# someguynamedjosh/raytrace

Measured on AMD Instinct MI355X. Metric: Mrays/s at 1920x1080 spp=64 (rays actually traced: primary + shadow + diffuse), higher is better.
Workload: dtype f32

## Files before the change

### include/rt_abi.h

```cpp
#ifndef RT_ABI_H
#define RT_ABI_H

#include <stddef.h>
#include <stdint.h>

#ifdef __cplusplus
extern "C" {
#endif

#define RT_CHUNK_SIZE        64
#define RT_MAX_CHUNK_LOD     6
#define RT_ROOT_CHUNK_SIZE   4
#define RT_ROOT_BLOCK_SIZE   256
#define RT_SLICE_SIZE        16
#define RT_SHADER_GROUP_SIZE 8
#define RT_PIXEL_SPREAD      16
#define RT_NOISE_SIZE        512
#define RT_NOISE_BYTES       (512 * 512 * 4)
#define RT_LIGHTING_SCALE    16.0f
#define RT_TRACE_LIMIT       2048
#define RT_NORMAL_AIR        16
#define RT_DEPTH_AIR         0xFFFF
#define RT_MAX_DEPTH         16

// ... 253 lines not shown
typedef struct RtPointLight {
    float    position[3];  float    radius;
    float    color[3];     uint32_t reserved;
} RtPointLight;
int rt_add_lights(RtContext* ctx, const RtUniforms* u, const RtPointLight* lights, uint32_t count);
int rt_add_lights_async(RtContext* ctx, const RtUniforms* u, const RtPointLight* lights_dev, uint32_t count);

int rt_shadow_entities(RtContext* ctx, const RtUniforms* u, const RtDrawBox* boxes, uint32_t nboxes, const RtDrawStamp* models,
                       uint32_t nmodels, float strength);
int rt_shadow_entities_async(RtContext* ctx, const RtUniforms* u, const RtDrawBox* boxes_dev, uint32_t nboxes, const RtDrawStamp* models,
                             uint32_t nmodels, float strength);

int rt_generate_world(RtContext* ctx, uint64_t seed, const int64_t window_lo[3]);
int rt_generate_slice(RtContext* ctx, uint64_t seed, int axis, const int64_t window_lo[3]);

int rt_get_info(RtContext* ctx, RtInfo* out);

uint64_t rt_samples_per_launch(uint64_t lane_bytes, uint64_t npix, uint64_t spp, const char* env_batch);

int rt_upload_noise(RtContext* ctx, const uint8_t* rgba8);

int rt_draw_frame(RtContext* ctx, const RtUniforms* uniforms);

int rt_sync(RtContext* ctx);

int rt_readback(RtContext* ctx, int buffer_id, void* dst, size_t bytes);

size_t rt_buffer_bytes(RtContext* ctx, int buffer_id);

void* rt_device_ptr(RtContext* ctx, int buffer_id);

int rt_set_stream(RtContext* ctx, void* hip_stream);

int rt_tile_count(RtContext* ctx);
int rt_tile_capacity(RtContext* ctx);

int rt_untile(RtContext* ctx, int buffer_id, const void* gathered_dev, int world, void* frame_dev);

void*  rt_gbuffer_ptr(RtContext* ctx);
size_t rt_gbuffer_bytes(RtContext* ctx);
size_t rt_gbuffer_offset(RtContext* ctx, int buffer_id);
int rt_untile_gbuffer(RtContext* ctx, const void* gathered_dev, int world, void* const* frames_dev);

int rt_denoise(RtContext* ctx, int faithful);

int rt_finalize(RtContext* ctx);

int rt_comm_unique_id(void* id_out, size_t bytes);
int rt_comm_init_rank(RtContext* ctx, const void* id, size_t bytes, void** comm_out);
int rt_comm_init_all(int ndev, const int* devices, void** comms_out);
int rt_comm_destroy(void* comm);
int rt_gather_gbuffer(RtContext* ctx, void* comm, int root, void* const* frames_dev, int overlapped);
void* rt_frame_ptr(RtContext* ctx, int buffer_id);
int rt_frame_readback(RtContext* ctx, int buffer_id, void* dst, size_t bytes);

int rt_denoise_planes(RtContext* ctx, void* lighting_rgba16, const void* depth_r16, const void* normal_r8, int faithful);
int rt_finalize_planes(RtContext* ctx, const void* albedo_rgba8, const void* emission_rgba8, const void* fog_rgba8,
                       const void* lighting_rgba16, const void* depth_r16, void* out_bgra8);

typedef struct RtDenoiseParams {
    uint32_t struct_size;
    int32_t  faithful;
    int32_t  weight_by_count;
    uint32_t settle[6];
    uint32_t reserved[3];
} RtDenoiseParams;
int rt_denoise_history(RtContext* ctx, const RtDenoiseParams* params);
int rt_denoise_planes_counted(RtContext* ctx, void* lighting_rgba16, const void* depth_r16, const void* normal_r8,
                              const uint32_t* counts_dev, const RtDenoiseParams* params);

int rt_kernel_in_use(RtContext* ctx);

#define RT_SELFTEST_DENOISE_DIVISION 1
#define RT_SELFTEST_SCENE_MAPS 2
int rt_selftest(RtContext* ctx, int which, uint64_t* result);

int rt_reset_accumulation(RtContext* ctx);
int rt_get_accumulation(RtContext* ctx, uint32_t* frames, uint32_t* samples);
int rt_read_history(RtContext* ctx, uint32_t* counts, size_t bytes);
int rt_edit_boxes_pending(RtContext* ctx, uint32_t* boxes, uint32_t* overflowed);
int rt_slabs_pending(RtContext* ctx, uint32_t* slabs, uint32_t* overflowed);
int rt_read_slab_boxes(RtContext* ctx, float* boxes, uint32_t* count);

int rt_get_counters(RtContext* ctx, RtCounters* out);
int rt_reset_counters(RtContext* ctx);
int rt_get_timing(RtContext* ctx, RtTiming* out);
int rt_get_gather_timing(RtContext* ctx, float* ms_sum, uint32_t* calls);

#define RT_ABI_VERSION_MAJOR 1
#define RT_ABI_VERSION_MINOR 3
uint32_t rt_abi_version(void);

#ifdef __cplusplus
}
#endif
#endif
```

### raytrace_amd/_lib.py

```python
import ctypes as C
import os

from .abi import RtConfig, RtCounters, RtDenoiseParams, RtInfo, RtShapeEdit, RtStampPlace, RtTiming, RtUniforms, RtVoxelEdit

HERE = os.path.dirname(os.path.abspath(__file__))
LIB_AMD_PATH = os.environ.get("RT_AMD_LIB") or os.path.join(HERE, "librt_amd.so")
LIB_HOST_PATH = os.path.join(HERE, "librt_host.so")

ABI_SYMBOLS = (
    "rt_create", "rt_destroy", "rt_last_error", "rt_upload_world", "rt_upload_slice", "rt_slice_staging", "rt_upload_noise",
    "rt_draw_frame", "rt_sync", "rt_readback", "rt_buffer_bytes", "rt_device_ptr", "rt_set_stream",
    "rt_tile_count", "rt_tile_capacity", "rt_untile", "rt_gbuffer_ptr", "rt_gbuffer_bytes", "rt_gbuffer_offset",
    "rt_untile_gbuffer", "rt_denoise", "rt_finalize", "rt_denoise_planes", "rt_finalize_planes", "rt_kernel_in_use", "rt_get_counters", "rt_reset_counters", "rt_get_timing",
    "rt_abi_version",
    "rt_comm_unique_id", "rt_comm_init_rank", "rt_comm_init_all", "rt_comm_destroy", "rt_gather_gbuffer", "rt_frame_ptr",
    "rt_frame_readback", "rt_selftest", "rt_get_info", "rt_samples_per_launch", "rt_get_gather_timing",
    "rt_reset_accumulation", "rt_get_accumulation", "rt_edit_voxels", "rt_read_box",
    "rt_trace_rays", "rt_trace_rays_async", "rt_pick_pixels", "rt_generate_world", "rt_generate_slice", "rt_read_history",
    "rt_edit_boxes_pending", "rt_slabs_pending", "rt_read_slab_boxes", "rt_probe_light", "rt_probe_light_async",
    "rt_denoise_history", "rt_denoise_planes_counted", "rt_sweep_boxes", "rt_sweep_boxes_async",
    "rt_edit_shapes", "rt_draw_boxes", "rt_draw_boxes_async", "rt_add_lights", "rt_add_lights_async",
    "rt_stamp_create", "rt_stamp_capture", "rt_stamp_info", "rt_stamp_read", "rt_stamp_destroy", "rt_edit_stamps",
    "rt_draw_stamps", "rt_draw_stamps_async", "rt_shadow_entities", "rt_shadow_entities_async",
)

_amd = None
_host = None


class NativeLibraryMissing(ImportError):
    pass


def amd():
    global _amd
    if _amd is None:
        if not os.path.exists(LIB_AMD_PATH):
            raise NativeLibraryMissing(
                "%s not found: the HIP extension is required (run `python -m raytrace_amd.build`); "
                "there is no CPU fallback" % LIB_AMD_PATH)
        lib = C.CDLL(LIB_AMD_PATH, mode=C.RTLD_GLOBAL)
        P = C.c_void_p
        lib.rt_create.argtypes = [C.POINTER(RtConfig), C.POINTER(P)]
        lib.rt_create.restype = C.c_int
        lib.rt_destroy.argtypes = [P]
        lib.rt_destroy.restype = None
        lib.rt_last_error.argtypes = [P]
        lib.rt_last_error.restype = C.c_char_p
        lib.rt_upload_world.argtypes = [P, P, P]
        lib.rt_upload_slice.argtypes = [P, C.c_int, C.c_int, P, P]
        lib.rt_slice_staging.argtypes = [P, C.POINTER(P), C.POINTER(P)]
        lib.rt_upload_noise.argtypes = [P, P]
        lib.rt_draw_frame.argtypes = [P, C.POINTER(RtUniforms)]
        lib.rt_sync.argtypes = [P]
        lib.rt_readback.argtypes = [P, C.c_int, P, C.c_size_t]
        lib.rt_buffer_bytes.argtypes = [P, C.c_int]
        lib.rt_buffer_bytes.restype = C.c_size_t
        lib.rt_device_ptr.argtypes = [P, C.c_int]
        lib.rt_device_ptr.restype = P
        lib.rt_set_stream.argtypes = [P, P]
        lib.rt_tile_count.argtypes = [P]
        lib.rt_tile_capacity.argtypes = [P]
        lib.rt_untile.argtypes = [P, C.c_int, P, C.c_int, P]
        lib.rt_gbuffer_ptr.argtypes = [P]
        lib.rt_gbuffer_ptr.restype = P
        lib.rt_gbuffer_bytes.argtypes = [P]
        lib.rt_gbuffer_bytes.restype = C.c_size_t
        lib.rt_gbuffer_offset.argtypes = [P, C.c_int]
        lib.rt_gbuffer_offset.restype = C.c_size_t
        lib.rt_untile_gbuffer.argtypes = [P, P, C.c_int, P]
        lib.rt_untile_gbuffer.restype = C.c_int
        lib.rt_denoise.argtypes = [P, C.c_int]
        lib.rt_finalize.argtypes = [P]
        lib.rt_denoise_planes.argtypes = [P, P, P, P, C.c_int]
        lib.rt_finalize_planes.argtypes = [P, P, P, P, P, P, P]
        lib.rt_denoise_history.argtypes = [P, C.POINTER(RtDenoiseParams)]
        lib.rt_denoise_history.restype = C.c_int
        lib.rt_denoise_planes_counted.argtypes = [P, P, P, P, P, C.POINTER(RtDenoiseParams)]
        lib.rt_denoise_planes_counted.restype = C.c_int
        lib.rt_kernel_in_use.argtypes = [P]
        lib.rt_kernel_in_use.restype = C.c_int
        lib.rt_get_counters.argtypes = [P, C.POINTER(RtCounters)]
        lib.rt_reset_counters.argtypes = [P]
        lib.rt_get_timing.argtypes = [P, C.POINTER(RtTiming)]
        lib.rt_get_info.argtypes = [P, C.POINTER(RtInfo)]
        lib.rt_get_info.restype = C.c_int
        lib.rt_abi_version.restype = C.c_uint32
        lib.rt_samples_per_launch.argtypes = [C.c_uint64, C.c_uint64, C.c_uint64, C.c_char_p]
        lib.rt_samples_per_launch.restype = C.c_uint64
        lib.rt_get_gather_timing.argtypes = [P, C.POINTER(C.c_float), C.POINTER(C.c_uint32)]
        lib.rt_get_gather_timing.restype = C.c_int
        lib.rt_comm_unique_id.argtypes = [P, C.c_size_t]
        lib.rt_comm_init_rank.argtypes = [P, P, C.c_size_t, C.POINTER(P)]
        lib.rt_comm_init_all.argtypes = [C.c_int, C.POINTER(C.c_int), C.POINTER(P)]
        lib.rt_comm_destroy.argtypes = [P]
        lib.rt_gather_gbuffer.argtypes = [P, P, C.c_int, P, C.c_int]
        lib.rt_frame_ptr.argtypes = [P, C.c_int]
        lib.rt_frame_ptr.restype = P
        lib.rt_frame_readback.argtypes = [P, C.c_int, P, C.c_size_t]
        lib.rt_frame_readback.restype = C.c_int
        lib.rt_selftest.argtypes = [P, C.c_int, C.POINTER(C.c_uint64)]
        lib.rt_selftest.restype = C.c_int
        lib.rt_reset_accumulation.argtypes = [P]
        lib.rt_reset_accumulation.restype = C.c_int
        lib.rt_get_accumulation.argtypes = [P, C.POINTER(C.c_uint32), C.POINTER(C.c_uint32)]
        lib.rt_get_accumulation.restype = C.c_int
        lib.rt_read_history.argtypes = [P, P, C.c_size_t]
        lib.rt_read_history.restype = C.c_int
        lib.rt_edit_boxes_pending.argtypes = [P, C.POINTER(C.c_uint32), C.POINTER(C.c_uint32)]
        lib.rt_edit_boxes_pending.restype = C.c_int
        lib.rt_slabs_pending.argtypes = [P, C.POINTER(C.c_uint32), C.POINTER(C.c_uint32)]
        lib.rt_slabs_pending.restype = C.c_int
        lib.rt_read_slab_boxes.argtypes = [P, P, C.POINTER(C.c_uint32)]
        lib.rt_read_slab_boxes.restype = C.c_int
        lib.rt_edit_voxels.argtypes = [P, C.POINTER(RtVoxelEdit), C.c_uint32]
        lib.rt_edit_voxels.restype = C.c_int
        lib.rt_edit_shapes.argtypes = [P, C.POINTER(RtShapeEdit), C.c_uint32]
        lib.rt_edit_shapes.restype = C.c_int
        lib.rt_stamp_create.argtypes = [P, C.POINTER(C.c_int32), P, P, C.POINTER(C.c_uint32)]
        lib.rt_stamp_capture.argtypes = [P, C.POINTER(C.c_int32), C.POINTER(C.c_int32), C.c_uint32, C.POINTER(C.c_uint32)]
        lib.rt_stamp_info.argtypes = [P, C.c_uint32, C.POINTER(C.c_int32)]
        lib.rt_stamp_read.argtypes = [P, C.c_uint32, P, P]
        lib.rt_stamp_destroy.argtypes = [P, C.c_uint32]
        lib.rt_edit_stamps.argtypes = [P, C.POINTER(RtStampPlace), C.c_uint32]
        for name in ("rt_stamp_create", "rt_stamp_capture", "rt_stamp_info", "rt_stamp_read", "rt_stamp_destroy", "rt_edit_stamps"):
            getattr(lib, name).restype = C.c_int
        lib.rt_read_box.argtypes = [P, C.c_int, C.c_int, C.c_int, C.c_int, C.c_int, C.c_int, P, P]
        lib.rt_read_box.restype = C.c_int
        lib.rt_trace_rays.argtypes = [P, P, C.c_uint32, C.POINTER(C.c_int32), P]
        lib.rt_trace_rays.restype = C.c_int
        lib.rt_trace_rays_async.argtypes = [P, P, C.c_uint32, C.POINTER(C.c_int32), P]
        lib.rt_trace_rays_async.restype = C.c_int
        lib.rt_pick_pixels.argtypes = [P, C.POINTER(RtUniforms), P, C.c_uint32, P]
        lib.rt_pick_pixels.restype = C.c_int
        lib.rt_probe_light.argtypes = [P, C.POINTER(RtUniforms), P, C.c_uint32, C.c_uint32, C.c_int32, P]
        lib.rt_probe_light.restype = C.c_int
        lib.rt_probe_light_async.argtypes = [P, C.POINTER(RtUniforms), P, C.c_uint32, C.c_uint32, C.c_int32, P]
        lib.rt_probe_light_async.restype = C.c_int
        lib.rt_sweep_boxes.argtypes = [P, P, C.c_uint32, C.POINTER(C.c_int32), P]
        lib.rt_sweep_boxes.restype = C.c_int
        lib.rt_sweep_boxes_async.argtypes = [P, P, C.c_uint32, C.POINTER(C.c_int32), P]
        lib.rt_sweep_boxes_async.restype = C.c_int
        lib.rt_draw_boxes.argtypes = [P, C.POINTER(RtUniforms), P, P, C.c_uint32]
        lib.rt_draw_boxes.restype = C.c_int
        lib.rt_draw_boxes_async.argtypes = [P, C.POINTER(RtUniforms), P, P, C.c_uint32]
        lib.rt_draw_boxes_async.restype = C.c_int
        lib.rt_draw_stamps.argtypes = [P, C.POINTER(RtUniforms), P, P, C.c_uint32]
        lib.rt_draw_stamps.restype = C.c_int
        lib.rt_draw_stamps_async.argtypes = [P, C.POINTER(RtUniforms), P, P, C.c_uint32]
        lib.rt_draw_stamps_async.restype = C.c_int
        lib.rt_shadow_entities.argtypes = [P, C.POINTER(RtUniforms), P, C.c_uint32, P, C.c_uint32, C.c_float]
        lib.rt_shadow_entities.restype = C.c_int
        lib.rt_shadow_entities_async.argtypes = [P, C.POINTER(RtUniforms), P, C.c_uint32, P, C.c_uint32, C.c_float]
        lib.rt_shadow_entities_async.restype = C.c_int
        lib.rt_add_lights.argtypes = [P, C.POINTER(RtUniforms), P, C.c_uint32]
        lib.rt_add_lights.restype = C.c_int
        lib.rt_add_lights_async.argtypes = [P, C.POINTER(RtUniforms), P, C.c_uint32]
        lib.rt_add_lights_async.restype = C.c_int
        lib.rt_generate_world.argtypes = [P, C.c_uint64, C.POINTER(C.c_int64)]
        lib.rt_generate_world.restype = C.c_int
        lib.rt_generate_slice.argtypes = [P, C.c_uint64, C.c_int, C.POINTER(C.c_int64)]
        lib.rt_generate_slice.restype = C.c_int
        for name in ("rt_comm_unique_id", "rt_comm_init_rank", "rt_comm_init_all", "rt_comm_destroy", "rt_gather_gbuffer"):
            getattr(lib, name).restype = C.c_int
        for name in ("rt_upload_world", "rt_upload_slice", "rt_slice_staging", "rt_upload_noise", "rt_draw_frame", "rt_sync", "rt_readback",
                     "rt_set_stream", "rt_tile_count", "rt_tile_capacity", "rt_untile", "rt_untile_gbuffer", "rt_denoise", "rt_finalize",
                     "rt_denoise_planes", "rt_finalize_planes", "rt_get_counters",
                     "rt_reset_counters", "rt_get_timing"):
            getattr(lib, name).restype = C.c_int
        _amd = lib
    return _amd


def host():
    global _host
    if _host is None:
        amd()
        if not os.path.exists(LIB_HOST_PATH):
            raise NativeLibraryMissing("%s not found (run `python -m raytrace_amd.build`)" % LIB_HOST_PATH)
        lib = C.CDLL(os.environ.get("RT_HOST_LIB") or LIB_HOST_PATH)
        P = C.c_void_p
        lib.rth_material_pack.argtypes = [C.c_int]
        lib.rth_material_pack.restype = C.c_uint32
        lib.rth_material_unpack.argtypes = [C.c_uint32, P, P]
        lib.rth_material_get.argtypes = [C.c_int, P, P, P]
        lib.rth_pack_chunk.argtypes = [P, P, P]
        lib.rth_generate_region.argtypes = [C.c_uint64, P, P]
        lib.rth_generate_region_r.argtypes = [C.c_uint64, C.c_int, P, P]
        lib.rth_region_from_ids.argtypes = [P, P, P]
        lib.rth_heightmap.argtypes = [C.c_long, C.c_long, C.c_uint64, P]
        lib.rth_copy_3d_u32.argtypes = [P] * 7
        lib.rth_copy_3d_auto_clip_u32.argtypes = [P, C.c_int, P, P, C.c_int]
        lib.rth_copy_3d_bounded_auto_clip_u32.argtypes = [P] * 7
        lib.rth_fill_slice_3d_auto_clip_u8.argtypes = [C.c_uint8, P, C.c_int, P, P]
        lib.rth_chunk_codec_available.restype = C.c_int
        lib.rth_chunk_file_name.argtypes = [C.c_long, C.c_long, C.c_long, P]
        lib.rth_chunk_write.argtypes = [C.c_char_p, P, P]
        lib.rth_chunk_read.argtypes = [C.c_char_p, P, P]
        lib.rth_chunk_storage_new.argtypes = [C.c_char_p, C.c_uint64]
        lib.rth_chunk_storage_new.restype = P
        lib.rth_chunk_storage_free.argtypes = [P]
        lib.rth_chunk_storage_free.restype = None
        lib.rth_chunk_storage_borrow.argtypes = [P, C.c_long, C.c_long, C.c_long, P, P]
        lib.rth_chunk_storage_stats.argtypes = [P, P, P]
        lib.rth_tum_new.argtypes = [C.c_uint64]
        lib.rth_tum_new.restype = P
        lib.rth_tum_new_r.argtypes = [C.c_uint64, C.c_int]
        lib.rth_tum_new_r.restype = P
        lib.rth_tum_free.argtypes = [P]
        lib.rth_tum_free.restype = None
        lib.rth_tum_request.argtypes = [P, C.c_int, C.c_int]
# ... 55 lines not shown
```

### raytrace_amd/csrc/api/api_context.hip

```cpp
#include <new>

#include "rt_context.hpp"

using namespace rta;

namespace rta __attribute__((visibility("hidden"))) {

thread_local std::string g_create_error = "";

rtd::Scene scene_of(const RtContext* c) {
    rtd::Scene s;
    s.mine = c->d_mine_sw; s.mat = c->d_mat_sw; s.coarse = c->d_coarse; s.noise = c->d_noise;
    s.brick = c->d_brick ? reinterpret_cast<const uint8_t*>(c->d_brick) : reinterpret_cast<const uint8_t*>(c->d_coarse);
    return s;
}

rtd::Planes planes_of(void* const* planes) {
    rtd::Planes p;
    p.lighting_rgba16 = (uint16_t*)planes[RT_BUF_LIGHTING_RGBA16];
    p.depth_r16 = (uint16_t*)planes[RT_BUF_DEPTH_R16UI];
    p.normal_r8 = (uint8_t*)planes[RT_BUF_NORMAL_R8UI];
    p.albedo_rgba8 = (uint32_t*)planes[RT_BUF_ALBEDO_RGBA8];
    p.emission_rgba8 = (uint32_t*)planes[RT_BUF_EMISSION_RGBA8];
    p.fog_rgba8 = (uint32_t*)planes[RT_BUF_FOG_RGBA8];
    p.lighting_f32 = (float*)planes[RT_BUF_LIGHTING_F32];
    p.fog_f32 = (float*)planes[RT_BUF_FOG_F32];
    p.depth_f32 = (float*)planes[RT_BUF_DEPTH_F32];
    return p;
}

hipError_t join_lanes_into(RtContext* c, hipStream_t st) {
    for (int l = 0; l < c->nlanes; l++) {
        Lane& ln = c->lanes[l];
        if (ln.stream == st || !ln.stream) continue;
        hipError_t e = hipEventRecord(ln.ev_join, ln.stream);
        if (e == hipSuccess) e = hipStreamWaitEvent(st, ln.ev_join, 0);
        if (e != hipSuccess) return e;
    }
    return hipSuccess;
}
hipError_t fence_lanes_after(RtContext* c, hipStream_t st) {
    if (c->nlanes < 2) return hipSuccess;
    hipError_t e = hipEventRecord(c->ev_fence, st);
    for (int l = 0; l < c->nlanes && e == hipSuccess; l++)
        if (c->lanes[l].stream != st) e = hipStreamWaitEvent(c->lanes[l].stream, c->ev_fence, 0);
    return e;
}
hipError_t sync_lanes(RtContext* c) {
    hipError_t e = hipStreamSynchronize(c->stream);
    if (e == hipSuccess && c->query_stream) e = hipStreamSynchronize(c->query_stream);
    for (int l = 0; l < c->nlanes && e == hipSuccess; l++)
        if (c->lanes[l].stream && c->lanes[l].stream != c->stream) e = hipStreamSynchronize(c->lanes[l].stream);
    return e;
}

void invalidate_prepass(RtContext* c) {
    for (FrameSlot& fs : c->slots) fs.prepass_valid = false;
}

void plane_written(RtContext* c, const void* ptr) {
    const uint8_t* q = static_cast<const uint8_t*>(ptr);
    for (int sl = 0; sl < c->nslots; sl++)
        for (int b = 0; b < RT_BUF_COUNT; b++) {
            if (b == RT_BUF_FINAL_BGRA8) continue;
            const uint8_t* base = static_cast<const uint8_t*>(c->slots[sl].planes[b]);
            if (base && q >= base && q < base + c->plane_pixels * kBytesPerPixel[b]) c->slots[sl].prepass_valid = false;
        }
}

}

constexpr uint64_t kDefaultLightBytes = 16ull << 30;
uint64_t rt_light_budget_bytes(const char* env_gib) {
    uint64_t light_bytes = kDefaultLightBytes;
    size_t free_b = 0, total_b = 0;
    if (hipMemGetInfo(&free_b, &total_b) == hipSuccess) { if ((uint64_t)free_b / 10u < light_bytes) light_bytes = (uint64_t)free_b / 10u; }
    else (void)hipGetLastError();
    uint64_t gib = 0;
    if (parse_knob(env_gib, 1, 128, &gib)) light_bytes = gib << 30;
    return light_bytes;
}
extern "C" uint64_t rt_samples_per_launch(uint64_t lane_bytes, uint64_t npix, uint64_t spp, const char* env_batch) {
    if (npix == 0) npix = 1;
    uint64_t B = lane_bytes / (sizeof(rtd::PathLight) * npix);
    if (B > (1ull << 31) / npix) B = (1ull << 31) / npix;
    parse_knob(env_batch, 1, (long long)B - 1, &B);
    if (B < 1) B = 1;
    if (B > spp) B = spp;
    return B;
}

namespace {

int create_device(RtContext* c) {
    RT_HIP(c, hipSetDevice(c->device));
    hipDeviceProp_t prop;
    RT_HIP(c, hipGetDeviceProperties(&prop, c->device));
    c->num_cus = prop.multiProcessorCount > 0 ? prop.multiProcessorCount : 256;
    int reserve = 0;
    if (env_int("RT_RESERVE_CUS", 1, c->num_cus - 1, &reserve)) c->num_cus -= reserve;
    RT_HIP(c, new_stream(c, &c->own_stream));
    c->stream = c->own_stream;
    c->lanes[0].stream = c->own_stream;
    for (hipEvent_t* ev : {&c->ev_frame0, &c->ev_frame1}) RT_HIP(c, new_event(c, ev, hipEventDefault));
    RT_HIP(c, dev_alloc(c, &c->d_mine_sw, c->vox)); RT_HIP(c, dev_alloc(c, &c->d_mat_sw, c->vox));
    RT_HIP(c, dev_alloc(c, &c->d_coarse, (size_t)rtd::kCoarseWords));
    if (c->logr > 8 && getenv("RT_BRICK_MAP")) RT_HIP(c, dev_alloc(c, &c->d_brick, c->vox / 128u / 4u));
    RT_HIP(c, dev_alloc(c, &c->d_noise, (size_t)RT_NOISE_SIZE * RT_NOISE_SIZE));
    RT_HIP(c, dev_alloc(c, &c->d_flag, 4));
    RT_HIP(c, dev_alloc(c, &c->d_counters, 1));
    RT_HIP(c, hipMemset(c->d_counters, 0, sizeof(rtd::DevCounters)));
    return RT_OK;
}

int create_slots(RtContext* c) {
    if (c->nlanes == 2) RT_HIP(c, new_stream(c, &c->lanes[1].stream));
    for (int l = 0; l < c->nlanes; l++) RT_HIP(c, new_event(c, &c->lanes[l].ev_join));
    for (hipEvent_t* ev : {&c->ev_fence, &c->ev_world.ev, &c->ev_query.ev, &c->ev_gather.ev}) RT_HIP(c, new_event(c, ev));
    size_t off = 0;
    for (int b = 0; b <= RT_BUF_FOG_RGBA8; b++) {
        c->gbuffer_offset[b] = off;
        off += (c->plane_pixels * kBytesPerPixel[b] + 255) / 256 * 256;
    }
    c->gbuffer_bytes = off;
    for (int sl = 0; sl < c->nslots; sl++) {
        FrameSlot& fs = c->slots[sl];
        uint8_t* block = nullptr;
        RT_HIP(c, dev_alloc(c, &block, off));
        RT_HIP(c, hipMemset(block, 0, off));
        fs.gbuffer = block;
        for (int b = 0; b <= RT_BUF_FOG_RGBA8; b++) fs.planes[b] = block + c->gbuffer_offset[b];
        for (int b = RT_BUF_FOG_RGBA8 + 1; b < RT_BUF_COUNT; b++) {
            uint8_t* p = nullptr;
            RT_HIP(c, dev_alloc(c, &p, c->plane_pixels * kBytesPerPixel[b]));
            RT_HIP(c, hipMemset(p, 0, c->plane_pixels * kBytesPerPixel[b]));
            fs.planes[b] = p;
        }
        for (hipEvent_t* ev : {&fs.ev_prepass, &fs.ev_acc, &fs.ev_tail.ev}) RT_HIP(c, new_event(c, ev));
    }
    c->cur_slot = 0;
    c->gbuffer = c->slots[0].gbuffer;
    for (int b = 0; b < RT_BUF_COUNT; b++) c->planes[b] = c->slots[0].planes[b];
    return RT_OK;
}

int create_persistent(RtContext* c) {
    const RtConfig& cfg = c->cfg;
    const size_t stack_words = (size_t)4 * c->num_cus * 1024 * (size_t)(cfg.depth > 1 ? cfg.depth - 1 : 1);
    for (int l = 0; l < c->nlanes; l++) {
        Lane& ln = c->lanes[l];
        RT_HIP(c, dev_alloc(c, &ln.cursor, kCursorWords));
        RT_HIP(c, hipMemset(ln.cursor, 0, kCursorWords * sizeof(uint32_t)));
        ln.cursor_clean = true;
        RT_HIP(c, dev_alloc(c, &ln.pstack, stack_words));
    }
    for (int sl = 0; sl < c->nslots; sl++) {
        FrameSlot& fs = c->slots[sl];
        RT_HIP(c, dev_alloc(c, &fs.wl_count, 2 * kWlSetWords));
        RT_HIP(c, hipMemset(fs.wl_count, 0, 2 * kWlSetWords * sizeof(uint32_t)));
        fs.wl_clean[0] = fs.wl_clean[1] = true;
        RT_HIP(c, dev_alloc(c, &fs.worklist, (size_t)c->npix_pad));
        RT_HIP(c, dev_alloc(c, &fs.phit, (size_t)c->npix_pad));
        RT_HIP(c, dev_alloc(c, &fs.pacc, (size_t)c->npix_pad));
    }
    RT_HIP(c, dev_alloc(c, &c->sphere_lut, (size_t)65536));
    RT_HIP(c, dev_alloc(c, &c->sun_lut, (size_t)2 * 65536));
    RT_HIP(c, dev_alloc(c, &c->dif_lut, (size_t)4 * 6 * 65536));
    const uint64_t np = c->npix_pad ? c->npix_pad : 1;
    c->light_budget_bytes = rt_light_budget_bytes(getenv("RT_PERSIST_LIGHT_GIB"));
    uint64_t B = rt_samples_per_launch(c->light_budget_bytes / (uint64_t)c->nlanes, np, (uint64_t)cfg.spp, getenv("RT_PERSIST_BATCH"));
    for (int l = 0; l < c->nlanes; l++) {
        for (;;) {
            const hipError_t e = dev_alloc(c, &c->lanes[l].ppl, (size_t)np * B);
            if (e == hipSuccess) break;
            if (e != hipErrorOutOfMemory || B == 1 || l > 0) RT_HIP(c, e);
            (void)hipGetLastError();
            B = (B + 1) / 2;
        }
    }
    c->persist_batch = (uint32_t)B;
    if (cfg.flags & RT_FLAG_ACCUMULATE) {
        RT_HIP(c, dev_alloc(c, &c->d_accum, (size_t)c->npix_pad));
        RT_HIP(c, new_event(c, &c->ev_accum.ev));
    }
    if (c->reproject) {
        c->d_hist_sum[0] = c->d_accum;
        RT_HIP(c, dev_alloc(c, &c->d_hist_sum[1], (size_t)c->npix_pad));
        for (int h = 0; h < 2; h++) {
            RT_HIP(c, dev_alloc(c, &c->d_hist_rec[h], (size_t)c->npix_pad));
            RT_HIP(c, hipMemset(c->d_hist_rec[h], 0, (size_t)c->npix_pad * sizeof(uint2)));
        }
    }
    if (c->stream_history) {
        RT_HIP(c, dev_alloc(c, &c->d_slab_masks, (size_t)rtd::kSlabSlots * rtd::kSlabSlotWords));
        RT_HIP(c, dev_alloc(c, &c->d_slab_boxes, 1));
        RT_HIP(c, hipMemset(c->d_slab_boxes, 0, sizeof(rtd::SlabBoxes)));
    }
    RT_HIP(c, rtd::launch_sphere_lut(c->sphere_lut, c->own_stream));
    RT_HIP(c, rtd::launch_dif_lut(c->sphere_lut, c->dif_lut, c->own_stream));
    RT_HIP(c, hipStreamSynchronize(c->own_stream));
    return RT_OK;
}

int create_wavefront(RtContext* c) {
    WavefrontState& w = c->wave;
    uint64_t target = 4u << 20;
    env_int("RT_BATCH_PATHS", 1, LLONG_MAX, &target);
    uint64_t B = c->npix_pad ? target / c->npix_pad : 1;
    if (B < 1) B = 1;
    if (B > (uint64_t)c->cfg.spp) B = (uint64_t)c->cfg.spp;
    w.batch_samples = (uint32_t)B;
    uint64_t cap64 = (uint64_t)c->npix_pad * B;
    if (cap64 >= (1ull << 31)) return fail(c, RT_ERR_INVALID_ARG, "rt_create: batch too large");
    w.cap = (uint32_t)cap64;
    const size_t cap = w.cap;
    rtd::ShadeArgs& sa = w.shade;
    RT_HIP(c, dev_alloc(c, &sa.qox, cap)); RT_HIP(c, dev_alloc(c, &sa.qoy, cap)); RT_HIP(c, dev_alloc(c, &sa.qoz, cap));
    RT_HIP(c, dev_alloc(c, &sa.qdx, 2 * cap)); RT_HIP(c, dev_alloc(c, &sa.qdy, 2 * cap)); RT_HIP(c, dev_alloc(c, &sa.qdz, 2 * cap));
    RT_HIP(c, dev_alloc(c, &sa.qid, cap));
    rtd::TraceArgs& ta = w.trace;
    RT_HIP(c, dev_alloc(c, &ta.hx, cap)); RT_HIP(c, dev_alloc(c, &ta.hy, cap)); RT_HIP(c, dev_alloc(c, &ta.hz, cap));
    RT_HIP(c, dev_alloc(c, &ta.hinfo, cap));
    RT_HIP(c, dev_alloc(c, &ta.sunres, cap)); RT_HIP(c, dev_alloc(c, &sa.pnormal, cap)); RT_HIP(c, dev_alloc(c, &sa.pstate, cap));
    RT_HIP(c, dev_alloc(c, &sa.pdx, cap)); RT_HIP(c, dev_alloc(c, &sa.pdy, cap)); RT_HIP(c, dev_alloc(c, &sa.pdz, cap));
    RT_HIP(c, dev_alloc(c, &sa.plx, cap)); RT_HIP(c, dev_alloc(c, &sa.ply, cap)); RT_HIP(c, dev_alloc(c, &sa.plz, cap));
    RT_HIP(c, dev_alloc(c, &sa.sunbits, cap));
    RT_HIP(c, dev_alloc(c, &sa.stack, cap * (size_t)(c->cfg.depth > 1 ? c->cfg.depth - 1 : 1)));
    RT_HIP(c, dev_alloc(c, &w.acc, (size_t)c->npix_pad));
    RT_HIP(c, dev_alloc(c, &w.ctrl, (size_t)2 * (RT_MAX_DEPTH + 2)));
    ta.qox = sa.qox; ta.qoy = sa.qoy; ta.qoz = sa.qoz; ta.qdx = sa.qdx; ta.qdy = sa.qdy; ta.qdz = sa.qdz; ta.qid = sa.qid;
    sa.hx = ta.hx; sa.hy = ta.hy; sa.hz = ta.hz; sa.hinfo = ta.hinfo; sa.sunres = ta.sunres;
    ta.qcap = sa.qcap = sa.npaths_cap = w.cap;
    ta.npix_pad = sa.npix_pad = c->npix_pad;
    ta.refill_threshold = w.refill_threshold;
    ta.counters = sa.counters = c->d_counters;
    return RT_OK;
}
}

extern "C" {

uint32_t rt_abi_version(void) { return ((uint32_t)RT_ABI_VERSION_MAJOR << 16) | (uint32_t)RT_ABI_VERSION_MINOR; }

const char* rt_last_error(RtContext* ctx) { return ctx ? ctx->err.c_str() : g_create_error.c_str(); }

int rt_create(const RtConfig* cfg, RtContext** out) {
    if (out) *out = nullptr;
    if (!cfg || !out) return fail(nullptr, RT_ERR_INVALID_ARG, "rt_create: null argument");
    if (cfg->struct_size != sizeof(RtConfig)) return fail(nullptr, RT_ERR_INVALID_ARG, "rt_create: RtConfig.struct_size mismatch");
    if (cfg->width <= 0 || cfg->height <= 0 || cfg->width > 16384 || cfg->height > 16384)
        return fail(nullptr, RT_ERR_INVALID_ARG, "rt_create: width/height out of range");
    if (cfg->region != 256 && cfg->region != 512 && cfg->region != 1024)
        return fail(nullptr, RT_ERR_INVALID_ARG, "rt_create: region must be 256 (the reference), 512 or 1024");
    if (cfg->region != 256 && cfg->kernel == RT_KERNEL_WAVEFRONT)
        return fail(nullptr, RT_ERR_INVALID_ARG, "rt_create: the split wavefront baseline supports region 256 only");
    if (cfg->spp < 1 || cfg->spp > RT_NOISE_BYTES) return fail(nullptr, RT_ERR_INVALID_ARG, "rt_create: spp out of range");
    if (cfg->depth < 0 || cfg->depth > RT_MAX_DEPTH) return fail(nullptr, RT_ERR_INVALID_ARG, "rt_create: depth out of range");
    if (cfg->tile_world < 1 || cfg->tile_rank < 0 || cfg->tile_rank >= cfg->tile_world)
        return fail(nullptr, RT_ERR_INVALID_ARG, "rt_create: bad tile_rank/tile_world");
    if (cfg->kernel < RT_KERNEL_DEFAULT || cfg->kernel > RT_KERNEL_FRAME || cfg->kernel == 4  ||
        cfg->kernel == 6 )
        return fail(nullptr, RT_ERR_INVALID_ARG, "rt_create: unknown kernel");
    if ((cfg->flags & RT_FLAG_ACCUMULATE) && (cfg->kernel == RT_KERNEL_MEGA || cfg->kernel == RT_KERNEL_WAVEFRONT))
        return fail(nullptr, RT_ERR_UNIMPLEMENTED, "rt_create: RT_FLAG_ACCUMULATE needs RT_KERNEL_DEFAULT, FRAME, PATHS or PERSISTENT (not the baselines)");
    if (cfg->flags & RT_FLAG_REPROJECT) {
        if (!(cfg->flags & RT_FLAG_ACCUMULATE))
            return fail(nullptr, RT_ERR_INVALID_ARG, "rt_create: RT_FLAG_REPROJECT needs RT_FLAG_ACCUMULATE");
        if (cfg->history_cap < 0 || cfg->history_cap > 65535)
            return fail(nullptr, RT_ERR_INVALID_ARG, "rt_create: history_cap must be 0 (the default, 32) or 1..65535");
        if (cfg->edit_radius < 0 || cfg->edit_radius > 64)
            return fail(nullptr, RT_ERR_INVALID_ARG, "rt_create: edit_radius must be 0 (an edit restarts the history) or 1..64");
        if (cfg->stream_history != 0 && cfg->stream_history != 1)
            return fail(nullptr, RT_ERR_INVALID_ARG, "rt_create: stream_history must be 0 (a slab restarts the history) or 1");
        if (cfg->stream_history == 1 && cfg->edit_radius < 1)
            return fail(nullptr, RT_ERR_INVALID_ARG, "rt_create: stream_history = 1 needs edit_radius in 1..64 (its near test uses it)");
        if (cfg->spp != 1 || cfg->tile_world != 1)
            return fail(nullptr, RT_ERR_UNIMPLEMENTED, "rt_create: RT_FLAG_REPROJECT needs one-sample whole frames (spp == 1, tile_world == 1)");
    }

// ... 232 lines not shown
```

### raytrace_amd/csrc/api/api_frame.hip

```cpp
#include "rt_context.hpp"

using namespace rta;

namespace rta __attribute__((visibility("hidden"))) {

void resolve_route(RtContext* c) {
    Route& r = c->route;
    if (r.family != RT_KERNEL_PERSISTENT) { r.in_use = r.family; return; }
    const RtConfig& cfg = c->cfg;
    const int kernel = cfg.kernel;
    const bool cache = (cfg.flags & RT_FLAG_CACHE_PRIMARY) != 0;
    const uint32_t spp = (uint32_t)cfg.spp, B = c->persist_batch;
    const uint64_t npix = c->npix_pad;
    rtd::Frame f{};
    f.depth = cfg.depth; f.logr = c->logr;
    const bool small = spp == 1u ? npix < c->frame_crossover
                                 : npix * spp * (uint64_t)(cfg.depth > 1 ? cfg.depth : 1) < c->frame_crossover_multi;
    r.frame = (cache || spp == 1u) && rtd::launch_frame_ok(f) && spp <= B && !((cfg.flags & RT_FLAG_ACCUMULATE) && spp > 1u) &&
              (kernel == RT_KERNEL_FRAME || (kernel == RT_KERNEL_DEFAULT && small));
    if (cache && kernel != RT_KERNEL_PERSISTENT)
        r.paths_from = kernel != RT_KERNEL_DEFAULT ? 0u : npix == 0 ? UINT32_MAX : (uint32_t)((kPathsCrossover + npix - 1) / npix);
    r.direct = spp == 1u && (!r.on_paths(1) || rtd::launch_paths_direct_ok(f));
    r.threshold_persist = c->persist_threshold ? c->persist_threshold : 32u;
    r.threshold_paths = c->persist_threshold ? c->persist_threshold : (cfg.depth > 4 && c->region == 256) ? 40u : 36u;
// ... 91 lines not shown
    FrameSlot* fs = nullptr;
    rtd::Planes pl{};
    bool one_lane = false;
    Lane* L0 = nullptr;
    hipStream_t st0 = nullptr;
    hipStream_t tail = nullptr;
    uint32_t* wlc = nullptr;
    bool reuse = false;
    bool accum = false, accum_cont = false;
    uint32_t key[16] = {};
    uint64_t accum_n = 0;
    float4* accum_multi = nullptr;
    int temporal_mode = rtd::TEMPORAL_RESTART;
    uint32_t nbox = 0;
    rtd::TemporalBox boxes[rtd::kTemporalMaxBoxes];
    uint32_t nslab = 0;
    int32_t lr_prev[3] = {}, lr[3] = {};
};

rtd::TemporalBox world_box(const EditBox& b, const int32_t lr[3], int region) {
    rtd::TemporalBox w;
    const int64_t R = region;
    for (int k = 0; k < 3; k++) {
        const int64_t base = (int64_t)lr[k] - R / 2;
        const int64_t lo = base + ((((int64_t)b.lo[k] - lr[k]) % R) + R) % R, hi = base + ((((int64_t)b.hi[k] - lr[k]) % R) + R) % R;
        w.lo[k] = (float)(lo <= hi ? lo : base);
        w.hi[k] = (float)(lo <= hi ? hi + 1 : base + R);
    }
    return w;
}

hipError_t frame_begin(RtContext* c, PersistFrame& p, const RtUniforms* u, bool frame_events) {
    p.count = (c->cfg.flags & RT_FLAG_COUNTERS) != 0;
    p.cache = (c->cfg.flags & RT_FLAG_CACHE_PRIMARY) != 0;
    p.nl = c->user_stream ? 1 : c->nlanes;
    p.nsl = c->user_stream ? 1 : c->nslots;
    hipError_t e = hipSuccess;
    if (c->frame_recorded) e = c->slots[c->cur_slot].ev_tail.record(c->stream);
    p.si = p.nsl == 2 ? (int)(c->frames_drawn & 1u) : 0;
    p.fs = &c->slots[p.si];
    p.pl = planes_of(p.fs->planes);
    p.one_lane = p.nsl == 1 && (uint32_t)c->cfg.spp <= c->persist_batch;
    p.L0 = &c->lanes[p.one_lane ? 0u : c->path_launches % (uint64_t)p.nl];
    p.st0 = p.tail = p.L0->stream;
    accum_key_of(u, p.key);
    p.reuse = c->prepass_reuse && p.cache && !c->route.frame && !p.count && c->d_accum == nullptr && !c->reproject &&
              (c->cfg.flags & (RT_FLAG_ACCUMULATE | RT_FLAG_REPROJECT)) == 0 && p.fs->prepass_valid &&
              memcmp(p.key, p.fs->prepass_key, sizeof(p.key)) == 0;
    p.wlc = p.fs->wl_count + kWlSetWords * (size_t)(p.fs->wl_parity ^ (p.reuse ? 1 : 0));
    const uint32_t spp = (uint32_t)c->cfg.spp;
    p.accum = c->d_accum != nullptr;
    if (c->edit_overflow) c->accum_valid = false;
    p.nbox = c->edit_nbox;
    for (uint32_t b = 0; b < p.nbox; b++) p.boxes[b] = world_box(c->edit_boxes[b], u->lr, c->region);
    c->edit_nbox = 0;
    c->edit_overflow = false;
    if (c->slab_overflow) c->accum_valid = false;
    p.nslab = c->slab_pending;
    memcpy(p.lr_prev, &c->accum_key[13], 12); memcpy(p.lr, u->lr, 12);
    c->slab_pending = 0;
    c->slab_overflow = false;
    c->slab_boxes_drawn = false;
    p.accum_cont = p.accum && c->accum_valid && memcmp(p.key, c->accum_key, sizeof(p.key)) == 0 && c->accum_samples + spp <= (1ull << 24);
    p.accum_n = p.accum_cont ? c->accum_samples + spp : spp;
    p.accum_multi = p.accum && spp > 1u ? c->d_accum : nullptr;
    if (c->reproject) {
        const bool still = p.accum_cont;
        const bool same_camera = memcmp(p.key, c->accum_key, sizeof(p.key)) == 0;
        if (still) p.temporal_mode = rtd::TEMPORAL_STILL;
        else if (c->accum_valid && !same_camera && p.key[0] == c->accum_key[0]) p.temporal_mode = rtd::TEMPORAL_MOVED;
        else p.temporal_mode = rtd::TEMPORAL_RESTART;
        if (p.temporal_mode != rtd::TEMPORAL_RESTART && p.nbox > 0u) p.temporal_mode = rtd::TEMPORAL_MOVED_BOXES;
        if (p.temporal_mode != rtd::TEMPORAL_RESTART && p.nslab > 0u) p.temporal_mode = rtd::TEMPORAL_MOVED_SLABS;
        if (p.temporal_mode != rtd::TEMPORAL_RESTART && p.temporal_mode != rtd::TEMPORAL_STILL) {
            p.accum_cont = true;
            p.accum_n = (c->accum_samples < c->history_cap ? c->accum_samples : (uint64_t)c->history_cap) + 1u;
        }
    }
    if (e == hipSuccess) e = p.fs->ev_tail.wait(p.st0);
    if (e == hipSuccess && frame_events) e = hipEventRecord(c->ev_frame0, p.st0);
    return e;
}

hipError_t frame_prepass(RtContext* c, PersistFrame& p) {
    FrameSlot& fs = *p.fs;
    const bool prepass_clears = c->primary_version == 2 && c->npix_pad != 0;
    hipError_t e = hipSuccess;
    fs.prepass_valid = false;
    if (!fs.wl_clean[fs.wl_parity]) e = hipMemsetAsync(p.wlc, 0, kWlClearWords * sizeof(uint32_t), p.st0);
    fs.wl_clean[fs.wl_parity] = false;
    LaunchTimer t(c, 1, p.st0);
    rtd::PrimaryArgs pr{};
    pr.phit = fs.phit;
    pr.worklist = fs.worklist; pr.wl_count = p.wlc; pr.tile_cursor = p.wlc + 32; pr.acc = fs.pacc; pr.counters = c->d_counters;
    const bool clear_cursors = prepass_clears && !p.L0->cursor_clean;
    pr.zero_words = prepass_clears ? fs.wl_count + kWlSetWords * (size_t)(fs.wl_parity ^ 1) : nullptr; pr.zero_count = (uint32_t)kWlClearWords;
    pr.zero_words2 = clear_cursors ? p.L0->cursor : nullptr; pr.zero_count2 = (uint32_t)kCursorWords;
    rtd::Frame fpre = p.f;
    if (p.accum_multi) fpre.spp = 1;
    if (e == hipSuccess) e = rtd::launch_primary(scene_of(c), fpre, p.pl, pr, p.count, c->primary_version, c->num_cus, p.st0);
    if (e == hipSuccess && p.accum_multi) e = c->ev_accum.wait_elsewhere(p.st0);
    if (e == hipSuccess && p.accum_multi)
        e = rtd::launch_accumulate_frame(p.f, p.pl, c->d_accum, c->npix_pad, p.accum_cont, (int)p.accum_n, c->cfg.spp, true, p.st0);
    if (prepass_clears && e == hipSuccess) { fs.wl_clean[fs.wl_parity ^ 1] = true; p.L0->cursor_clean = true; }
    fs.wl_parity ^= 1;
    if (e == hipSuccess) { fs.prepass_valid = true; memcpy(fs.prepass_key, p.key, sizeof(p.key)); }
    return e;
}

hipError_t frame_tables(RtContext* c, PersistFrame& p) {
    const float lut_key[6] = {p.f.sunangle[0], p.f.sunangle[1], p.f.sunangle[2], p.f.sunlight[0], p.f.sunlight[1], p.f.sunlight[2]};
    if (c->cfg.depth < 1 || (c->lut_valid && memcmp(lut_key, c->lut_key, sizeof(lut_key)) == 0)) return hipSuccess;
    hipError_t e = p.nl == 2 ? join_lanes_into(c, p.st0) : hipSuccess;
    {
        LaunchTimer t(c, 1, p.st0);
        if (e == hipSuccess) e = rtd::launch_sun_lut(p.f, c->sun_lut, p.st0);
        if (e == hipSuccess) e = rtd::launch_sky_lut(p.f, c->dif_lut, p.st0);
    }
    if (e == hipSuccess && p.nl == 2) e = fence_lanes_after(c, p.st0);
    c->lut_valid = e == hipSuccess;
    memcpy(c->lut_key, lut_key, sizeof(lut_key));
    return e;
}

hipError_t frame_one_launch(RtContext* c, PersistFrame& p) {
    if (p.nsl == 2) c->path_launches++;
    rtd::FrameArgs fa{};
    fa.threshold = c->frame_threshold; fa.tiles_per_group = c->frame_tiles; fa.sun_lut = c->sun_lut; fa.dif_lut = c->dif_lut; fa.pl = p.L0->ppl; fa.counters = c->d_counters;
    if (getenv("RT_DEBUG_WAVE_DUMP") && (size_t)c->ntiles_local * 32u <= (size_t)4 * c->num_cus * 1024 * sizeof(uint32_t))
        fa.dbg_waves = reinterpret_cast<unsigned long long*>(c->lanes[0].pstack);
    LaunchTimer t(c, 0, p.st0);
    return rtd::launch_frame(scene_of(c), p.f, p.pl, fa, p.count, c->num_cus, p.st0);
}

hipError_t frame_path_batches(RtContext* c, PersistFrame& p) {
    const Route& r = c->route;
    FrameSlot& fs = *p.fs;
    const uint32_t spp = (uint32_t)c->cfg.spp, B = c->persist_batch;
    hipError_t e = hipSuccess;
    if (p.nl == 2 && spp > B) e = hipEventRecord(fs.ev_prepass, p.st0);
    for (uint32_t s0 = 0; s0 < spp && e == hipSuccess; s0 += B) {
        const uint32_t ns = spp - s0 < B ? spp - s0 : B;
        Lane* L = &c->lanes[p.one_lane ? 0u : c->path_launches % (uint64_t)p.nl];
        const hipStream_t st = L->stream;
        if (!p.one_lane) c->path_launches++;
        if (st != p.st0 && s0 == B) e = hipStreamWaitEvent(st, fs.ev_prepass, 0);
        if (e == hipSuccess && !L->cursor_clean) e = hipMemsetAsync(L->cursor, 0, kCursorWords * sizeof(uint32_t), st);
        L->cursor_clean = false;
        const bool to_paths = r.on_paths(ns);
        rtd::PersistArgs pa{};
        pa.cursor = L->cursor; pa.worklist = fs.worklist; pa.wl_count = p.wlc; pa.direct = r.direct ? 1u : 0u;
        pa.npix_pad = c->npix_pad; pa.sample0 = s0; pa.nsamples = ns; pa.chunk = c->persist_chunk;
        pa.threshold = to_paths ? r.threshold_paths : r.threshold_persist;
        pa.nthreads = (uint32_t)c->num_cus * 1024u; pa.stack = L->pstack;
        pa.phit = fs.phit;
        pa.sun_lut = c->sun_lut; pa.dif_lut = c->dif_lut;
        pa.pl = L->ppl; pa.counters = c->d_counters;
        const uint64_t record_bytes = (uint64_t)c->npix_pad * ns * sizeof(rtd::PathLight);
        const bool big_records = record_bytes > kStreamRecordBytes;
        const bool stream_st = c->pl_stream_mode < 0 ? big_records : (c->pl_stream_mode & 1) != 0;
        const bool stream_ld = c->pl_stream_mode < 0 ? big_records : (c->pl_stream_mode & 2) != 0;
        pa.pl_stream = stream_st ? 1u : 0u;
        if (e == hipSuccess) {
            LaunchTimer t(c, 0, st);
            e = to_paths ? rtd::launch_paths(scene_of(c), p.f, p.pl, pa, p.count, c->num_cus, st)
                         : rtd::launch_persist(scene_of(c), p.f, p.pl, pa, p.count, p.cache, 1, c->num_cus, st);
        }
        if (e == hipSuccess && !r.direct) {
            if (p.nl == 2 && s0 != 0) e = hipStreamWaitEvent(st, fs.ev_acc, 0);
            if (e == hipSuccess && p.accum_multi && !p.cache && s0 == 0) e = c->ev_accum.wait_elsewhere(st);
            {
                LaunchTimer t(c, 1, st);
                if (e == hipSuccess)
                    e = rtd::launch_accumulate_paths(p.f, p.pl, L->ppl, fs.worklist, p.wlc, c->npix_pad, ns, s0 == 0, s0 + B >= spp, p.cache,
                                                     stream_ld, fs.pacc, p.accum_multi, p.accum_cont, (int)p.accum_n, L->cursor,
                                                     (uint32_t)kCursorWords, st);
                if (e == hipSuccess && c->npix_pad != 0) L->cursor_clean = true;
            }
            if (e == hipSuccess && p.nl == 2 && s0 + B < spp) e = hipEventRecord(fs.ev_acc, st);
        }
        p.tail = st;
    }
    return e;
}

hipError_t frame_accumulate_tail(RtContext* c, PersistFrame& p) {
    hipError_t e = hipSuccess;
    if (c->cfg.spp == 1) {
        e = c->ev_accum.wait_elsewhere(p.tail);
        LaunchTimer t(c, 1, p.tail);
        if (e == hipSuccess && !c->reproject)
            e = rtd::launch_accumulate_frame(p.f, p.pl, c->d_accum, c->npix_pad, p.accum_cont, (int)p.accum_n, 1, false, p.tail);
        if (e == hipSuccess && c->reproject) {
            rtd::TemporalArgs ta{};
            const int prev = c->hist_cur, next = prev ^ 1;
            ta.prev_sum = c->d_hist_sum[prev]; ta.prev_rec = c->d_hist_rec[prev];
            ta.next_sum = c->d_hist_sum[next]; ta.next_rec = c->d_hist_rec[next];
            memcpy(ta.origin, &c->accum_key[1], 12); memcpy(ta.forward, &c->accum_key[4], 12);
            memcpy(ta.up, &c->accum_key[7], 12); memcpy(ta.right, &c->accum_key[10], 12);
            ta.cap = c->history_cap;
            if (p.temporal_mode == rtd::TEMPORAL_MOVED_SLABS) {
                e = rtd::launch_place_slab_boxes(c->d_slab_masks, p.nslab, p.lr_prev, p.lr, c->logr, c->d_slab_boxes, p.tail);
                ta.slab = c->d_slab_boxes;
                c->slab_boxes_drawn = e == hipSuccess;
            }
            if (p.temporal_mode == rtd::TEMPORAL_MOVED_BOXES || p.temporal_mode == rtd::TEMPORAL_MOVED_SLABS) {
                ta.nbox = p.nbox;
                memcpy(ta.box, p.boxes, sizeof(ta.box));
                ta.r2 = (float)(c->edit_radius * c->edit_radius);
                for (int k = 0; k < 3; k++) { ta.sun[k] = p.f.sunangle[k]; ta.inv_sun[k] = 1.0f / p.f.sunangle[k]; }
            }
            if (e == hipSuccess) e = rtd::launch_temporal_frame(p.f, p.pl, ta, p.temporal_mode, p.tail);
            c->hist_cur = next;
        }
    }
    if (e == hipSuccess && p.nl == 2) e = c->ev_accum.record(p.tail);
    return e;
}

void frame_publish(RtContext* c, const PersistFrame& p, hipError_t e) {
    if (e != hipSuccess) invalidate_prepass(c);
    if (p.accum) {
        c->accum_valid = e == hipSuccess;
        c->accum_frames = p.accum_cont ? c->accum_frames + 1u : 1u;
        c->accum_samples = p.accum_n;
        memcpy(c->accum_key, p.key, sizeof(p.key));
    }
    c->stream = p.tail;
    c->cur_slot = p.si;
    c->gbuffer = p.fs->gbuffer;
    for (int b = 0; b < RT_BUF_COUNT; b++) c->planes[b] = p.fs->planes[b];
    c->frames_drawn++;
}

int draw_persistent(RtContext* c, const rtd::Frame& f, const RtUniforms* u, bool frame_events) {
    PersistFrame p{f};
    hipError_t e = frame_begin(c, p, u, frame_events);
    if (e == hipSuccess && p.cache && !c->route.frame && !p.reuse) e = frame_prepass(c, p);
    if (e == hipSuccess) e = frame_tables(c, p);
    if (e == hipSuccess && c->route.frame) e = frame_one_launch(c, p);
    else if (e == hipSuccess && (!p.cache || c->cfg.depth >= 1)) e = frame_path_batches(c, p);
    if (e == hipSuccess && p.accum) e = frame_accumulate_tail(c, p);
    frame_publish(c, p, e);
    return e == hipSuccess ? RT_OK : fail(c, RT_ERR_HIP, std::string("persistent path: ") + hipGetErrorString(e));
}

}

extern "C" {

int rt_draw_frame(RtContext* ctx, const RtUniforms* u) {
    if (!ctx) return RT_ERR_INVALID_ARG;
    if (!u) return fail(ctx, RT_ERR_INVALID_ARG, "rt_draw_frame: null uniforms");
    if (!ctx->has_world || !ctx->has_noise) return fail(ctx, RT_ERR_NOT_READY, "rt_draw_frame: world and noise must be uploaded first");
    RT_HIP(ctx, hipSetDevice(ctx->device));
    const rtd::Frame f = frame_of(ctx, u);
    const bool count = (ctx->cfg.flags & RT_FLAG_COUNTERS) != 0;
    const bool frame_events = (ctx->cfg.flags & RT_FLAG_TIMING_ALL) == RT_FLAG_TIMING_ALL;
    int rc = RT_OK;
    if (ctx->route.family == RT_KERNEL_MEGA) {
        if (frame_events) RT_HIP(ctx, hipEventRecord(ctx->ev_frame0, ctx->stream));
        LaunchTimer t(ctx, 0);
        hipError_t e = rtd::launch_mega(scene_of(ctx), f, planes_of(ctx), ctx->d_counters, count, ctx->stream);
        if (e != hipSuccess) rc = fail(ctx, RT_ERR_HIP, std::string("launch_mega: ") + hipGetErrorString(e));
    } else if (ctx->route.family == RT_KERNEL_PERSISTENT) {
        rc = draw_persistent(ctx, f, u, frame_events);
    } else {
        if (frame_events) RT_HIP(ctx, hipEventRecord(ctx->ev_frame0, ctx->stream));
        rc = draw_wavefront(ctx, f);
    }
    if (frame_events) RT_HIP(ctx, hipEventRecord(ctx->ev_frame1, ctx->stream));
    ctx->frame_recorded = true;
    if (rc == RT_OK) ctx->drawn = true;
    if (count) { ctx->host_noise_base += (uint64_t)ctx->cfg.spp; ctx->host_frames++; }
    return rc;
}

int rt_reset_accumulation(RtContext* ctx) {
    if (!ctx) return RT_ERR_INVALID_ARG;
    restart_history(ctx);
    return RT_OK;
}

int rt_edit_boxes_pending(RtContext* ctx, uint32_t* boxes, uint32_t* overflowed) {
    if (!ctx) return RT_ERR_INVALID_ARG;
    if (!boxes || !overflowed) return fail(ctx, RT_ERR_INVALID_ARG, "rt_edit_boxes_pending: null pointer");
    *boxes = ctx->edit_nbox;
    *overflowed = ctx->edit_overflow ? 1u : 0u;
    return RT_OK;
}

int rt_slabs_pending(RtContext* ctx, uint32_t* slabs, uint32_t* overflowed) {
    if (!ctx) return RT_ERR_INVALID_ARG;
    if (!slabs || !overflowed) return fail(ctx, RT_ERR_INVALID_ARG, "rt_slabs_pending: null pointer");
    *slabs = ctx->slab_pending;
    *overflowed = ctx->slab_overflow ? 1u : 0u;
    return RT_OK;
}

int rt_read_slab_boxes(RtContext* ctx, float* boxes, uint32_t* count) {
    if (!ctx) return RT_ERR_INVALID_ARG;
    if (!ctx->stream_history) return fail(ctx, RT_ERR_INVALID_ARG, "rt_read_slab_boxes: the context was created without RtConfig.stream_history");
    if (!boxes || !count) return fail(ctx, RT_ERR_INVALID_ARG, "rt_read_slab_boxes: null pointer");
    RT_HIP(ctx, hipSetDevice(ctx->device));
    RT_HIP(ctx, sync_lanes(ctx));
    *count = 0;
    if (!ctx->slab_boxes_drawn) return RT_OK;
    rtd::SlabBoxes b;
    RT_HIP(ctx, hipMemcpy(&b, ctx->d_slab_boxes, sizeof(b), hipMemcpyDeviceToHost));
    *count = b.count <= rtd::kSlabMaxBoxes ? b.count : rtd::kSlabMaxBoxes;
    memcpy(boxes, b.box, (size_t)*count * sizeof(rtd::TemporalBox));
    return RT_OK;
}

int rt_get_accumulation(RtContext* ctx, uint32_t* frames, uint32_t* samples) {
    if (!ctx) return RT_ERR_INVALID_ARG;
    if (!frames || !samples) return fail(ctx, RT_ERR_INVALID_ARG, "rt_get_accumulation: null pointer");
    if (!ctx->drawn) { *frames = 0; *samples = 0; }
    else if (ctx->d_accum) { *frames = (uint32_t)ctx->accum_frames; *samples = (uint32_t)ctx->accum_samples; }
    else { *frames = 1; *samples = (uint32_t)ctx->cfg.spp; }
    return RT_OK;
}
// ... 16 lines not shown
```

### raytrace_amd/csrc/api/api_world.hip

```cpp
#include "rt_context.hpp"

using namespace rta;

namespace {

hipError_t world_change_begin(RtContext* c) {
    hipError_t e = join_lanes_into(c, c->stream);
    if (e == hipSuccess) e = c->ev_query.wait(c->stream);
    return e;
}
hipError_t world_change_end(RtContext* c) {
    hipError_t e = c->ev_world.record(c->stream);
    return e == hipSuccess ? fence_lanes_after(c, c->stream) : e;
}

hipError_t staging_claim(RtContext* c, StagingSet& s, size_t need, size_t alloc) {
    hipError_t e = c->upload_stream ? hipSuccess : new_stream(c, &c->upload_stream);
    for (hipEvent_t* ev : {&s.ev_copied.ev, &s.ev_applied.ev})
        if (e == hipSuccess && !*ev) e = new_event(c, ev);
    if (e == hipSuccess) e = s.ev_copied.host_wait();
    if (e == hipSuccess) s.ev_copied.forget();
    if (e != hipSuccess || need <= s.cap) return e;
    e = s.ev_applied.host_wait();
    return e == hipSuccess ? s.grow(c, need, alloc) : e;
// ... 334 lines not shown
    }
    e->used = true;
    *id_out = e->id;
    return RT_OK;
}

int rt_stamp_info(RtContext* ctx, uint32_t id, int32_t extent_out[3]) {
    if (!ctx) return RT_ERR_INVALID_ARG;
    const StampEntry* e = ctx->stamps.find(id);
    if (!e) return fail(ctx, RT_ERR_INVALID_ARG, "rt_stamp_info: unknown stamp id");
    if (!extent_out) return fail(ctx, RT_ERR_INVALID_ARG, "rt_stamp_info: null pointer");
    for (int k = 0; k < 3; k++) extent_out[k] = e->ext[k];
    return RT_OK;
}

int rt_stamp_read(RtContext* ctx, uint32_t id, uint32_t* materials, uint8_t* state) {
    if (!ctx) return RT_ERR_INVALID_ARG;
    StampEntry* e = ctx->stamps.find(id);
    if (!e) return fail(ctx, RT_ERR_INVALID_ARG, "rt_stamp_read: unknown stamp id");
    RT_HIP(ctx, hipSetDevice(ctx->device));
    RT_HIP(ctx, sync_lanes(ctx));
    e->used = false;
    if (materials) RT_HIP(ctx, hipMemcpy(materials, reinterpret_cast<const void*>(e->mats), e->voxels() * sizeof(uint32_t), hipMemcpyDeviceToHost));
    if (state) RT_HIP(ctx, hipMemcpy(state, reinterpret_cast<const void*>(e->state), e->voxels(), hipMemcpyDeviceToHost));
    return RT_OK;
}

int rt_stamp_destroy(RtContext* ctx, uint32_t id) {
    if (!ctx) return RT_ERR_INVALID_ARG;
    StampEntry* e = ctx->stamps.find(id);
    if (!e) return fail(ctx, RT_ERR_INVALID_ARG, "rt_stamp_destroy: unknown stamp id");
    RT_HIP(ctx, hipSetDevice(ctx->device));
    if (e->used) RT_HIP(ctx, sync_lanes(ctx));
    stamp_free(ctx, e);
    return RT_OK;
}

int rt_edit_stamps(RtContext* ctx, const RtStampPlace* places, uint32_t count) {
    if (!ctx) return RT_ERR_INVALID_ARG;
    if (count > kMaxStampPlaces) return fail(ctx, RT_ERR_INVALID_ARG, "rt_edit_stamps: more than 4096 placements in one call; nothing was applied");
    if (count == 0) return RT_OK;
    if (!places) return fail(ctx, RT_ERR_INVALID_ARG, "rt_edit_stamps: null places");
    if (!ctx->world_resident) return fail(ctx, RT_ERR_NOT_READY, "rt_edit_stamps: upload the full region first");
    const uint32_t bad = places_validate(ctx->stamps, places, count, ctx->logr);
    if (bad != count)
        return fail(ctx, RT_ERR_INVALID_ARG, "rt_edit_stamps: placement " + std::to_string(bad) +
                                                 " has an unknown stamp id, orient >= 48, where > 2, a non-zero reserved field or an at[k]"
                                                 " outside [-4R, 4R]; nothing was applied");
    const StampPlan plan = stamps_touched(ctx->shape_scratch, ctx->stamps, places, count, ctx->logr);
    if (plan.touched == 0u) return RT_OK;
    RT_HIP(ctx, hipSetDevice(ctx->device));
    StagingSet& s = ctx->edit_sets[ctx->edit_batches & 1u];
    const size_t cap = plan.need < ((size_t)64 << 10) ? ((size_t)64 << 10) : align16(plan.need + plan.need / 2u);
    RT_HIP(ctx, staging_claim(ctx, s, plan.need, cap));
    shapes_fill_chunks(ctx->shape_scratch, reinterpret_cast<uint32_t*>(s.host));
    stamp_fill_records(ctx->stamps, places, count, ctx->logr, reinterpret_cast<StampRecord*>(s.host + plan.off_recs));
    for (uint32_t i = 0; i < count; i++) ctx->stamps.find(places[i].stamp)->used = true;
    ctx->edit_batches++;
    if (ctx->edit_radius == 0u) {
        ctx->accum_valid = false;
    } else if (!ctx->edit_overflow) {
        if (ctx->edit_nbox + plan.boxes > rtd::kTemporalMaxBoxes) {
            ctx->edit_nbox = 0;
            ctx->edit_overflow = true;
        } else {
            ctx->edit_nbox += stamp_pending_boxes(ctx->stamps, places, count, ctx->logr, ctx->edit_boxes + ctx->edit_nbox);
        }
    }
    invalidate_prepass(ctx);
    RT_HIP(ctx, staging_send(ctx, s, plan.need));
    const uint32_t* d_chunks = reinterpret_cast<const uint32_t*>(s.dev);
    {
        LaunchTimer lt(ctx, 1);
        RT_HIP(ctx, rtd::launch_stamp_chunks(ctx->d_mine_sw, ctx->d_mat_sw, d_chunks, s.dev + plan.off_recs, count, plan.touched, ctx->logr, ctx->stream));
    }
    {
        LaunchTimer lt(ctx, 1);
        RT_HIP(ctx, rtd::launch_rebuild_chunk_maps(ctx->d_mine_sw, ctx->d_coarse, ctx->d_brick, d_chunks, plan.touched, ctx->logr, ctx->stream));
    }
    RT_HIP(ctx, staging_applied(ctx, s));
    return RT_OK;
}

int rt_read_box(RtContext* ctx, int x0, int y0, int z0, int ex, int ey, int ez, uint32_t* materials, uint8_t* minefield) {
    if (!ctx) return RT_ERR_INVALID_ARG;
    const int R = ctx->region;
    if (x0 < 0 || y0 < 0 || z0 < 0 || ex < 1 || ey < 1 || ez < 1 || ex > R - x0 || ey > R - y0 || ez > R - z0)
        return fail(ctx, RT_ERR_INVALID_ARG, "rt_read_box: box outside the region");
    if (!ctx->world_resident) return fail(ctx, RT_ERR_NOT_READY, "rt_read_box: no region uploaded");
    if (!materials && !minefield) return RT_OK;
    RT_HIP(ctx, hipSetDevice(ctx->device));
    RT_HIP(ctx, sync_lanes(ctx));
    const size_t plane = (size_t)ex * (size_t)ey;
    const int nz = (int)(((size_t)1 << 24) / plane >= (size_t)ez ? (size_t)ez : (((size_t)1 << 24) / plane > 0 ? ((size_t)1 << 24) / plane : 1));
    uint32_t* d_mat = nullptr; uint8_t* d_mine = nullptr;
    hipError_t e = hipSuccess;
    if (materials) e = hipMalloc((void**)&d_mat, plane * (size_t)nz * sizeof(uint32_t));
    if (e == hipSuccess && minefield) e = hipMalloc((void**)&d_mine, plane * (size_t)nz);
    for (int z = 0; z < ez && e == hipSuccess; z += nz) {
        const int n = ez - z < nz ? ez - z : nz;
        e = rtd::launch_read_box(ctx->d_mine_sw, ctx->d_mat_sw, ctx->logr, x0, y0, z0 + z, ex, ey, n, d_mat, d_mine, ctx->stream);
        if (e == hipSuccess && materials)
            e = hipMemcpyAsync(materials + plane * (size_t)z, d_mat, plane * (size_t)n * sizeof(uint32_t), hipMemcpyDeviceToHost, ctx->stream);
        if (e == hipSuccess && minefield)
            e = hipMemcpyAsync(minefield + plane * (size_t)z, d_mine, plane * (size_t)n, hipMemcpyDeviceToHost, ctx->stream);
        if (e == hipSuccess) e = hipStreamSynchronize(ctx->stream);
    }
    if (d_mat) (void)hipFree(d_mat);
    if (d_mine) (void)hipFree(d_mine);
    if (e != hipSuccess) return fail(ctx, e == hipErrorOutOfMemory ? RT_ERR_OOM : RT_ERR_HIP, std::string("rt_read_box: ") + hipGetErrorString(e));
    return RT_OK;
}

}
```

### raytrace_amd/csrc/api/rt_context.hpp

```cpp
#pragma once

#include <hip/hip_runtime.h>

#include <climits>
#include <cstdio>
#include <cstdlib>
#include <cstring>
#include <initializer_list>
#include <string>
#include <vector>

#include "../../../include/rt_abi.h"
#include "../../../include/rt_math.h"
#include "../rt_kernels.hpp"
#include "edit_binning.hpp"
#include "edit_shapes.hpp"
#include "edit_stamps.hpp"
#include "draw_stamps.hpp"

namespace rta __attribute__((visibility("hidden"))) {

constexpr size_t kBytesPerPixel[RT_BUF_COUNT] = {8, 2, 1, 4, 4, 4, 16, 16, 4, 4};

constexpr size_t kWlSetWords = 64, kWlClearWords = 33;
// ... 51 lines not shown
    size_t acquire(hipStream_t st, hipError_t* e) {
        *e = hipSuccess;
        if (used + 2 > kMaxTimerEvents) return npos;
        while (ev.size() < used + 2) {
            hipEvent_t n;
            if ((*e = hipEventCreate(&n)) != hipSuccess) return npos;
            ev.push_back(n);
        }
        const size_t idx = used;
        used += 2;
        *e = hipEventRecord(ev[idx], st);
        return idx;
    }
    hipError_t release(size_t idx, hipStream_t st) { return hipEventRecord(ev[idx + 1], st); }
    template <typename F>
    hipError_t drain(F&& each) {
        for (size_t i = 0; i + 1 < used; i += 2) {
            float ms = 0.0f;
            const hipError_t e = hipEventElapsedTime(&ms, ev[i], ev[i + 1]);
            if (e != hipSuccess) return e;
            each(i / 2, ms);
        }
        used = 0;
        return hipSuccess;
    }
};

struct Lane {
    hipStream_t stream = nullptr;
    uint32_t* cursor = nullptr;
    bool cursor_clean = false;
    uint32_t* pstack = nullptr;
    rtd::PathLight* ppl = nullptr;
    hipEvent_t ev_join = nullptr;
};
struct FrameSlot {
    void* planes[RT_BUF_COUNT] = {};
    void* gbuffer = nullptr;
    uint32_t* worklist = nullptr;
    float4* phit = nullptr;
    float4* pacc = nullptr;
    uint32_t* wl_count = nullptr;
    int wl_parity = 0;
    bool wl_clean[2] = {false, false};
    bool prepass_valid = false;
    uint32_t prepass_key[16] = {};
    void* denoise_work[2] = {nullptr, nullptr};
    hipEvent_t ev_prepass = nullptr;
    hipEvent_t ev_acc = nullptr;
    LatchEvent ev_tail;
};

struct WavefrontState {
    rtd::TraceArgs trace{};
    rtd::ShadeArgs shade{};
    float4* acc = nullptr;
    uint32_t* ctrl = nullptr;
    uint32_t batch_samples = 1;
    uint32_t cap = 0;
    uint32_t refill_threshold = 24;
};

}

struct __attribute__((visibility("hidden"))) RtContext {
    RtConfig cfg{};
    int device = 0;
    int num_cus = 256;
    int logr = 8;
    int region = RT_ROOT_BLOCK_SIZE;
    size_t vox = 0;
    hipStream_t own_stream = nullptr, stream = nullptr;
    bool user_stream = false;
    std::string err = "";
    bool has_world = false, has_noise = false;
    bool world_resident = false;

    std::vector<hipEvent_t> events;
    std::vector<hipStream_t> streams;

    uint8_t* d_mine_sw = nullptr; uint32_t* d_mat_sw = nullptr;
    uint32_t* d_coarse = nullptr; uint32_t* d_noise = nullptr; uint32_t* d_flag = nullptr;
    uint32_t* d_brick = nullptr;
    hipStream_t upload_stream = nullptr;
    rta::StagingSet slab_sets[2], edit_sets[2];
    uint64_t slabs = 0, edit_batches = 0;
    rta::EditBinning edit_binning;
    rta::ShapeScratch shape_scratch;
    rta::StampStore stamps;
    int32_t* d_heights = nullptr;

    int tiles_x = 0, tiles_y = 0, ntiles_total = 0, ntiles_local = 0, tile_capacity = 0;
    uint32_t npix_pad = 0;
    size_t plane_pixels = 0;

    void* planes[RT_BUF_COUNT] = {};
    void* gbuffer = nullptr;
    size_t gbuffer_offset[6] = {};
    size_t gbuffer_bytes = 0;
    rta::Lane lanes[2];
    int nlanes = 1;
    rta::FrameSlot slots[2];
    int nslots = 1;
    int cur_slot = 0;
    uint64_t frames_drawn = 0, path_launches = 0;
    hipEvent_t ev_fence = nullptr;
    rta::LatchEvent ev_gather;

    rta::Route route;

    rta::WavefrontState wave;
    float4* sphere_lut = nullptr;
    float4* sun_lut = nullptr;
    float4* dif_lut = nullptr;
    uint32_t persist_batch = 1;
    int pl_stream_mode = -1;
    uint32_t persist_chunk = 0;
    uint32_t persist_threshold = 0;
    uint64_t frame_crossover = rta::kFrameCrossover;
    uint64_t frame_crossover_multi = rta::kFrameCrossoverMulti;
    uint32_t frame_threshold = 0;
    uint32_t frame_tiles = 0;
    float lut_key[6] = {0, 0, 0, 0, 0, 0};
    bool lut_valid = false;
    int primary_version = 2;
    rtd::DevCounters* d_counters = nullptr;
    unsigned long long* d_selftest = nullptr;
    uint64_t host_noise_base = 0, host_frames = 0;

    hipEvent_t ev_frame0 = nullptr, ev_frame1 = nullptr;
    rta::TimingPool launch_times;
    std::vector<int> launch_kind;
    uint32_t timer_overflow = 0;
    bool frame_recorded = false;

    void* frame_planes[6] = {};
    uint8_t* gathered[2] = {nullptr, nullptr};
    uint8_t* stage[2] = {nullptr, nullptr};
    hipStream_t gather_stream = nullptr;
    hipEvent_t ev_ready[2] = {nullptr, nullptr};
    rta::LatchEvent ev_free[2];
    uint64_t gathers = 0;
    rta::TimingPool gather_times;

    std::vector<void*> allocs;
    uint64_t device_bytes = 0;
    uint64_t light_budget_bytes = 0;

    float4* d_accum = nullptr;
    bool accum_valid = false;
    bool prepass_reuse = true;
    uint32_t accum_key[16] = {};
    uint64_t accum_frames = 0, accum_samples = 0;
    bool drawn = false;
    rta::LatchEvent ev_accum;
    bool reproject = false;
    uint32_t history_cap = 32;
    float4* d_hist_sum[2] = {nullptr, nullptr};
    uint2* d_hist_rec[2] = {nullptr, nullptr};
    int hist_cur = 0;
    uint32_t edit_radius = 0;
    rta::EditBox edit_boxes[rtd::kTemporalMaxBoxes];
    uint32_t edit_nbox = 0;
    bool edit_overflow = false;
    bool stream_history = false;
    uint32_t* d_slab_masks = nullptr;
// ... 134 lines not shown
```

### raytrace_amd/csrc/rt_device.hpp

```cpp
#pragma once
#include <hip/hip_runtime.h>
#include <stdint.h>

#include "../../include/rt_abi.h"
#include "../../include/rt_math.h"

namespace rtd {

constexpr int kCoarsePerAxis = 64;
constexpr int kCoarseCount = kCoarsePerAxis * kCoarsePerAxis * kCoarsePerAxis;
constexpr int kCoarseWords = kCoarseCount / 8;
constexpr uint32_t kNibMixed = 15;
constexpr uint32_t kMaxStepValue = 30;

__device__ __forceinline__ uint32_t swizzled_index(int ix, int iy, int iz, int lb) {
    const uint32_t brick = ((uint32_t)(iz >> 2) << (2 * lb)) | ((uint32_t)(iy >> 2) << lb) | (uint32_t)(ix >> 2);
    return (brick << 6) | ((uint32_t)(iz & 3) << 4) | ((uint32_t)(iy & 3) << 2) | (uint32_t)(ix & 3);
}
__device__ __forceinline__ uint32_t coarse_index(int ix, int iy, int iz, int logr) {
    const int sh = logr - 6;
    return ((uint32_t)(iz >> sh) << 12) | ((uint32_t)(iy >> sh) << 6) | (uint32_t)(ix >> sh);
}

struct Scene {
    const uint8_t* mine;
    const uint32_t* mat;
    const uint32_t* coarse;
    const uint8_t* brick;
    const uint32_t* noise;
};

struct Frame {
    float origin[3], forward[3], up[3], right[3];
    float lr[3];
    float sunangle[3], sunlight[3];
    uint32_t seed;
    int width, height;
    int tiles_x, tiles_y;
    int tile_rank, tile_world;
    int ntiles_local;
    int spp, depth;
    int lr_zero;
    int logr;
    float region;
};

struct vec3 { float x, y, z; };
__device__ __forceinline__ vec3 v3(float x, float y, float z) { vec3 v = {x, y, z}; return v; }
__device__ __forceinline__ vec3 vadd(vec3 a, vec3 b) { return v3(a.x + b.x, a.y + b.y, a.z + b.z); }
__device__ __forceinline__ vec3 vsub(vec3 a, vec3 b) { return v3(a.x - b.x, a.y - b.y, a.z - b.z); }
__device__ __forceinline__ vec3 vscale(vec3 a, float s) { return v3(a.x * s, a.y * s, a.z * s); }
__device__ __forceinline__ vec3 vmul(vec3 a, vec3 b) { return v3(a.x * b.x, a.y * b.y, a.z * b.z); }
__device__ __forceinline__ vec3 vnormalize(vec3 v) { rtm_vec3 o = rtm_normalize3({v.x, v.y, v.z}); return v3(o.x, o.y, o.z); }
__device__ __forceinline__ float vlength(vec3 v) { return rtm_length3({v.x, v.y, v.z}); }
__device__ __forceinline__ vec3 vmix(vec3 a, vec3 b, float t) { return v3(rtm_mix(a.x, b.x, t), rtm_mix(a.y, b.y, t), rtm_mix(a.z, b.z, t)); }
__device__ __forceinline__ vec3 ld3(const float* p) { return v3(p[0], p[1], p[2]); }

struct PixelId { int px, py; bool inside; uint32_t out_index; };
__device__ __forceinline__ PixelId pixel_of_local(const Frame& f, uint32_t local_pixel) {
    uint32_t j = local_pixel >> 6, l = local_pixel & 63;
    uint32_t t = (uint32_t)f.tile_rank + j * (uint32_t)f.tile_world;
    PixelId p;
    p.px = (int)(t % (uint32_t)f.tiles_x) * 8 + (int)(l & 7);
    p.py = (int)(t / (uint32_t)f.tiles_x) * 8 + (int)(l >> 3);
    p.inside = p.px < f.width && p.py < f.height && j < (uint32_t)f.ntiles_local;
    p.out_index = f.tile_world == 1 ? (uint32_t)p.py * (uint32_t)f.width + (uint32_t)p.px : local_pixel;
    return p;
}

__device__ __forceinline__ uint32_t owning_workgroup(uint32_t p) { return (p / 128u) * 16u + (p % 16u); }

__device__ __forceinline__ uint32_t noise_texel(const Scene& sc, float cx, float cy) {
    float fx = rtm_floor(cx), fy = rtm_floor(cy);
    int ix = fx < 0.0f ? 0 : (fx > 511.0f ? 511 : (int)fx);
    int iy = fy < 0.0f ? 0 : (fy > 511.0f ? 511 : (int)fy);
    if (!(fx == fx)) ix = 0;
    if (!(fy == fy)) iy = 0;
    return sc.noise[iy * RT_NOISE_SIZE + ix];
}
__device__ __forceinline__ float unorm8(uint32_t texel, int channel) { return (float)((texel >> (8 * channel)) & 0xFFu) / 255.0f; }

struct NoiseOffset { float x, y; };
__device__ __forceinline__ NoiseOffset noise_offset_of(const Scene& sc, uint32_t seed, int px, int py) {
    uint32_t base = noise_texel(sc, (float)(seed % RT_NOISE_SIZE), (float)(seed / RT_NOISE_SIZE));
    NoiseOffset o;
    o.x = unorm8(base, 0) * 255.0f + (float)(owning_workgroup((uint32_t)px) * RT_SHADER_GROUP_SIZE);
    o.y = unorm8(base, 1) * 255.0f + (float)(owning_workgroup((uint32_t)py) * RT_SHADER_GROUP_SIZE);
    return o;
}
__device__ __forceinline__ uint32_t noise_value_texel(const Scene& sc, NoiseOffset o, int level) {
    float add = (float)(level - 1) * (2.0f / (float)RT_NOISE_SIZE);
    return noise_texel(sc, rtm_mod(o.x + add, (float)RT_NOISE_SIZE), rtm_mod(o.y + add, (float)RT_NOISE_SIZE));
}

__device__ __forceinline__ vec3 sample_sky(vec3 direction, vec3 sun_direction, vec3 sunlight, bool include_sun) {
    const vec3 bright_color = v3(0.5294f, 0.8275f, 0.9647f);
// ... 181 lines not shown
```

### raytrace_amd/csrc/rt_kernels.hpp

```cpp
#pragma once
#include <hip/hip_runtime.h>
#include <stdint.h>

#include <type_traits>

#include "rt_device.hpp"

namespace rtd {

template <typename Launch>
void launch_for_region(const Frame& f, Launch&& launch) {
    auto with = [&](auto L) {
        if (f.lr_zero != 0) launch(L, std::true_type{});
        else launch(L, std::false_type{});
    };
    if (f.logr == 8) with(std::integral_constant<int, 8>{});
    else if (f.logr == 9) with(std::integral_constant<int, 9>{});
    else with(std::integral_constant<int, 10>{});
}

struct TraceArgs {
    const float *qox, *qoy, *qoz, *qdx, *qdy, *qdz;
    const uint32_t* qid;
    const uint32_t* qcount;
// ... 9 lines not shown
};

struct ShadeArgs {
    float *qox, *qoy, *qoz, *qdx, *qdy, *qdz;
    uint32_t* qid;
    uint32_t* qcount_next;
    uint32_t qcap;
    uint32_t npaths;
    uint32_t npaths_cap;
    uint32_t npix_pad;
    uint32_t sample0;
    const float *hx, *hy, *hz;
    const uint32_t* hinfo;
    const uint8_t* sunres;
    float *pdx, *pdy, *pdz;
    uint8_t* pnormal;
    uint8_t* pstate;
    uint32_t* sunbits;
    uint32_t* stack;
    float *plx, *ply, *plz;
    DevCounters* counters;
};

struct PrimaryArgs {
    float4* phit;
    uint32_t* worklist;
    uint32_t* wl_count;
    uint32_t* tile_cursor;
    uint32_t* zero_words;
    uint32_t zero_count;
    uint32_t* zero_words2;
    uint32_t zero_count2;
    float4* acc;
    DevCounters* counters;
};
struct PathLight { float x, y, z; };
struct PersistArgs {
    uint32_t* cursor;
    const uint32_t* worklist;
    const uint32_t* wl_count;
    uint32_t npix_pad;
    uint32_t sample0, nsamples;
    uint32_t threshold;
    uint32_t rmin;
    uint32_t chunk;
    uint32_t nthreads;
    uint32_t direct;
    uint32_t pl_stream;
    uint32_t* stack;
    const float4* phit;
    const float4* sun_lut;
    const float4* dif_lut;
    PathLight* pl;
    DevCounters* counters;
};
struct FrameArgs {
    uint32_t threshold;
    uint32_t tiles_per_group;
    uint32_t pair_a;
    const float4* sun_lut;
    const float4* dif_lut;
    PathLight* pl;
    DevCounters* counters;
    unsigned long long* dbg_waves;
};
bool launch_frame_ok(const Frame& f);
hipError_t launch_frame(const Scene& sc, const Frame& f, const Planes& pl, FrameArgs a, bool count, int num_cus, hipStream_t st);
hipError_t launch_accumulate_paths(const Frame& f, const Planes& planes, const PathLight* pl, const uint32_t* worklist,
                                   const uint32_t* wl_count, uint32_t npix_pad, uint32_t nsamples, bool first_batch, bool last_batch,
                                   bool cache, bool stream, float4* acc, float4* accum, bool accum_continue, int accum_div,
                                   uint32_t* zero_words, uint32_t zero_count, hipStream_t st);
hipError_t launch_accumulate_frame(const Frame& f, const Planes& planes, float4* accum, uint32_t npix_pad, bool accum_continue, int n,
                                   int reps, bool finished_only, hipStream_t st);
hipError_t launch_sphere_lut(float4* lut, hipStream_t st);
hipError_t launch_dif_lut(const float4* sphere, float4* lut, hipStream_t st);
hipError_t launch_sun_lut(const Frame& f, float4* lut, hipStream_t st);
hipError_t launch_sky_lut(const Frame& f, float4* dif_lut, hipStream_t st);
hipError_t launch_primary(const Scene& sc, const Frame& f, const Planes& pl, const PrimaryArgs& a, bool count,
                          int version , int nworkgroups, hipStream_t st);
hipError_t launch_persist(const Scene& sc, const Frame& f, const Planes& pl, const PersistArgs& a, bool count, bool cache,
                          int version , int nworkgroups, hipStream_t st);

bool launch_paths_direct_ok(const Frame& f);
hipError_t launch_paths(const Scene& sc, const Frame& f, const Planes& pl, const PersistArgs& a, bool count, int nworkgroups,
                        hipStream_t st);

struct MapBoxes { uint3 cw0, cwn, bw0, bwn; };
MapBoxes map_boxes_region(int logr);
MapBoxes map_boxes_slab(int logr, int axis, int texel_offset);
hipError_t launch_build_maps(const uint8_t* mine_sw, uint32_t* coarse, uint32_t* brick ,
                             int logr, const MapBoxes& boxes, hipStream_t st);
hipError_t launch_flatten(const uint8_t* mine_lin, const uint32_t* mat_lin, uint8_t* mine_sw, uint32_t* mat_sw,
                          uint32_t* coarse, uint32_t* brick, uint32_t* bad_flag, int logr, hipStream_t st);
hipError_t launch_flatten_slab(const uint8_t* mine_slab, const uint32_t* mat_slab, uint8_t* mine_sw, uint32_t* mat_sw, uint32_t* coarse,
                               uint32_t* brick, int logr, int axis, int offset, hipStream_t st);
hipError_t launch_check_maps(const uint8_t* mine_sw, const uint32_t* coarse, const uint32_t* brick, int logr,
                             unsigned long long* mismatches, hipStream_t st);
hipError_t launch_read_box(const uint8_t* mine_sw, const uint32_t* mat_sw, int logr, int x0, int y0, int z0, int ex, int ey, int nz,
                           uint32_t* mat_out, uint8_t* mine_out, hipStream_t st);
hipError_t launch_rebuild_chunks(uint8_t* mine_sw, uint32_t* mat_sw, const uint32_t* chunks, const uint32_t* offs, const uint2* recs,
                                 uint32_t nchunks, int logr, hipStream_t st);
hipError_t launch_shape_chunks(uint8_t* mine_sw, uint32_t* mat_sw, const uint32_t* chunks, const void* shapes, uint32_t nshapes,
                               uint32_t nchunks, int logr, hipStream_t st);
hipError_t launch_stamp_chunks(uint8_t* mine_sw, uint32_t* mat_sw, const uint32_t* chunks, const void* recs, uint32_t nrecs,
                               uint32_t nchunks, int logr, hipStream_t st);
hipError_t launch_stamp_capture(const uint8_t* mine_sw, const uint32_t* mat_sw, int logr, int x0, int y0, int z0, int ex, int ey, int ez,
                                bool skip_air, uint32_t* mats_out, uint8_t* state_out, hipStream_t st);
hipError_t launch_stamp_clean(uint32_t* mats, const uint8_t* state, uint32_t n, hipStream_t st);
hipError_t launch_rebuild_chunk_maps(const uint8_t* mine_sw, uint32_t* coarse, uint32_t* brick, const uint32_t* chunks, uint32_t nchunks,
                                     int logr, hipStream_t st);
hipError_t launch_terrain(uint8_t* mine_sw, uint32_t* mat_sw, uint32_t* coarse, uint32_t* brick, int32_t* heights, int logr,
                          uint64_t seed, const int64_t lo[3], int axis, hipStream_t st);
hipError_t launch_mega(const Scene& sc, const Frame& f, const Planes& pl, DevCounters* cn, bool count, hipStream_t st);
hipError_t launch_trace(const Scene& sc, const Frame& f, const TraceArgs& a, bool primary, bool count, int nworkgroups, hipStream_t st);
hipError_t launch_shade0(const Scene& sc, const Frame& f, const ShadeArgs& a, const Planes& pl, bool count, hipStream_t st);
hipError_t launch_shadeN(const Scene& sc, const Frame& f, const ShadeArgs& a, int level, bool count, hipStream_t st);
hipError_t launch_accumulate(const float* plx, const float* ply, const float* plz, float4* acc, uint32_t npix_pad,
                             uint32_t nsamples, bool first_batch, hipStream_t st);
hipError_t launch_resolve(const Frame& f, const float4* acc, const Planes& pl, uint32_t npix_pad, hipStream_t st);
hipError_t launch_untile_strided(const void* gathered, size_t rank_stride, void* frame, int world, int capacity, int tiles_x,
                                 int tiles_y, int width, int height, int bpp, hipStream_t st);
hipError_t launch_untile(const void* gathered, void* frame, int world, int capacity, int tiles_x, int tiles_y, int width,
                         int height, int bpp, hipStream_t st);

struct QueryArgs {
    const float4* rays;
    const int2* xy;
    uint4* hits;
    uint32_t count;
};
hipError_t launch_query(const Scene& sc, const Frame& f, const QueryArgs& a, hipStream_t st);

constexpr uint64_t kProbeMaxPaths = 1ull << 26;
struct ProbeArgs {
    const uint4* probes;
    uint4* out;
    float4* scratch;
    uint32_t count, samples;
};
bool probe_sums_in_lds(uint32_t samples);
hipError_t launch_probe(const Scene& sc, const Frame& f, const ProbeArgs& a, bool pair, hipStream_t st);

struct SweepArgs {
    const uint4* sweeps;
    uint4* hits;
    uint32_t count;
    int32_t lr[3];
};
hipError_t launch_sweep(const Scene& sc, int logr, const SweepArgs& a, hipStream_t st);

struct DrawBoxesArgs {
    const uint4* boxes;
    const float4* lights;
    uint32_t count;
    int width, height;
    float origin[3], forward[3], up[3], right[3];
};
hipError_t launch_draw_boxes(const Planes& pl, const DrawBoxesArgs& a, hipStream_t st);

struct DrawStampsArgs {
    const uint4* recs;
    const float4* lights;
    uint32_t count;
    int width, height;
    float origin[3], forward[3], up[3], right[3];
};
hipError_t launch_draw_stamps(const Planes& pl, const DrawStampsArgs& a, hipStream_t st);

struct LightsArgs {
    const uint4* lights;
    uint32_t count;
};
hipError_t launch_add_lights(const Scene& sc, const Frame& f, const Planes& pl, const LightsArgs& a, hipStream_t st);

struct ShadowArgs {
    const uint4* boxes;
    const uint4* recs;
    uint32_t nboxes, nmodels;
    float strength;
};
// ... 40 lines not shown
```

### raytrace_amd/csrc/rt_paths.hip

```cpp
#include <hip/hip_runtime.h>

#include <type_traits>

#include "rt_device.hpp"
#include "rt_kernels.hpp"
#include "rt_pslot.hpp"

#ifndef RT_PATHS_STEPS_PER_CHECK
#define RT_PATHS_STEPS_PER_CHECK 3
#endif
#ifndef RT_PATHS_DRAIN_PARK
#define RT_PATHS_DRAIN_PARK 8
#endif
#ifndef RT_PATHS_SHADOW_REPS
#define RT_PATHS_SHADOW_REPS 0x3
#endif
#ifndef RT_PATHS_BRICK_MAP
#define RT_PATHS_BRICK_MAP 0
#endif

namespace rtd {
using namespace pslot;

template <bool COUNT, int STK, int LOGR, bool LRZ>
__global__ __launch_bounds__(1024) void k_paths(Scene sc, Frame f, Planes pl, PersistArgs a) {
    static_assert(LOGR == 8 || STK == 1, "the larger regions' tables leave no LDS for the albedo stack");
    constexpr bool LDS_ROWS = STK == 0 || STK == 2;
    constexpr int R = 1 << LOGR, LB = LOGR - 2;
    constexpr uint32_t kTabWords = swz_bytes<LOGR>() / 4u;
    __shared__ uint32_t s_coarse[kCoarseWords];
    __shared__ __attribute__((aligned(swz_bytes<LOGR>()))) uint32_t s_swz[3 * kTabWords];
    __shared__ float s_albedo[128];
    __shared__ uint32_t s_stack[LDS_ROWS ? 2 : 1][LDS_ROWS ? 3 : 1][LDS_ROWS ? 1024 : 1];
    const uint32_t nwork = *a.wl_count;
    const uint32_t nitems = nwork * a.nsamples;
    if (nitems == 0u) return;
    {
        const uint4* src = reinterpret_cast<const uint4*>(sc.coarse);
        uint4* dst = reinterpret_cast<uint4*>(s_coarse);
        for (uint32_t i = threadIdx.x; i < kCoarseWords / 4; i += 1024u) dst[i] = src[i];
        if (threadIdx.x < 128u) s_albedo[threadIdx.x] = (float)threadIdx.x / 127.0f;
        for (uint32_t i = threadIdx.x; i < 3u * kTabWords; i += 1024u) {
            const uint32_t ax = i / kTabWords, e = i % kTabWords, v = e & (uint32_t)(R - 1);
            const uint32_t word = ((v & 3u) << (2u * ax)) | ((v >> 2) << (6u + (uint32_t)LB * ax));
            s_swz[i] = (!LRZ && e == (uint32_t)R) ? kSwzBorder : word;
        }
    }
    __syncthreads();

    constexpr float half = (float)(R / 2);
    const uint8_t* s_nib = reinterpret_cast<const uint8_t*>(s_coarse);
    const uint32_t swz = (uint32_t)(uintptr_t)(lds_u32*)s_swz;
    const uint32_t lane = threadIdx.x & 63u;
    const uint32_t gtid = blockIdx.x * 1024u + threadIdx.x;
    const uint32_t threshold = a.threshold;
    const vec3 sunlight = ld3(f.sunlight);
    const uint32_t D = (uint32_t)f.depth;
    const uint32_t stack_levels = D > 1u ? D - 1u : 1u;
    const auto mine_rsrc = __builtin_amdgcn_make_buffer_rsrc(const_cast<uint8_t*>(sc.mine), (short)0, 1 << (3 * LOGR), 0x00020000);
    const auto brick_rsrc = __builtin_amdgcn_make_buffer_rsrc(const_cast<uint8_t*>(sc.brick), (short)0, 1 << (3 * LOGR - 7), 0x00020000);
    unsigned long long d_fetch = 0, d_fetch_cube = 0, d_fetch_brick = 0;

#ifdef RT_DIAG_WAVE_TIMES
    const unsigned long long t_wave0 = wall_clock64();
    unsigned long long t_exh = 0;
#endif
    PRay SA, FA, SB, FB;
    SA.px = SA.py = SA.pz = SA.ndx = SA.ndy = SA.lx = SA.ly = SA.lz = 0.0f; SA.ndz = -1.0f;
    SA.sx = SA.sy = SA.sz = 0u; SA.nk = (uint32_t)RT_TRACE_LIMIT;
    FA = SA; SB = SA; FB = SA;
    lanemask rSA = 0, rFA = 0, rSB = 0, rFB = 0;
    lanemask zFA = ~0ull, xyFA = 0, zFB = ~0ull, xyFB = 0;
    lanemask nul = 0, nul2 = 0;
    uint32_t looks = 0;
    PPath PA, PB;
    PA.st = PP_FINAL; PA.item = 0u; PA.ent = 7u << 16;
    PB = PA;

    bool exhausted = false;
    const uint32_t kChunk = a.chunk ? a.chunk : 128u;
    uint32_t chunk_next = 0, chunk_end = 0;
    uint32_t chunk_sb = 0, chunk_w = 0;
    uint32_t chunk_w0 = 0, chunk_nw = 1;
    const uint32_t home_grp = blockIdx.x & 7u;
    uint32_t grp_tries = 0;

    unsigned long long c_shadow = 0, c_dif = 0, c_iter = 0, c_hits = 0, c_sky = 0, c_limit = 0, c_border = 0, c_noise = 0;
    unsigned long long d_iters = 0, d_passf = 0, d_plf = 0, d_live = 0;

    auto lookup = [&](uint32_t vox) -> uint32_t {
        if (!LRZ && ps_border(vox)) return 0u;
        uint32_t nb, nsh;
        ps_nibble_of<LOGR, LRZ>(vox, &nb, &nsh);
        uint32_t st = (s_nib[nb] >> nsh) & 15u;
        if (LOGR > 8 && RT_PATHS_BRICK_MAP != 0 && st == kNibMixed) st = (sc.brick[vox >> 7] >> ((vox >> 4) & 4u)) & 15u;
        if (st == kNibMixed) st = sc.mine[vox];
        return st;
    };
    auto stop_kind = [&](uint32_t nk, uint32_t vox, bool consider) -> uint32_t {
        const uint32_t left = nk & 0xFFFFu;
        uint32_t kind = left == (uint32_t)RT_TRACE_LIMIT ? 2u : 0u;
        const bool at_limit = consider && left == 0u;
        if (__builtin_expect(__ballot(at_limit) != 0ull, 0)) {
            if (at_limit && lookup(vox) != 0u) kind = 1u;
        }
        return kind;
    };
    auto tally = [&](const PRay& r) {
        const uint32_t left = r.nk & 0xFFFFu;
        if (pr_outside<LOGR, LRZ>(r.px, r.py, r.pz, f.lr[0], f.lr[1], f.lr[2])) {
            c_iter += (uint32_t)RT_TRACE_LIMIT - left;
            c_sky++;
            int tx, ty, tz;
            if (!wrap_texel(v3(r.px, r.py, r.pz), (float)R, &tx, &ty, &tz)) c_border++;
        } else {
            const uint32_t kind = stop_kind(r.nk, pr_vox(r), true);
            c_iter += kind == 2u ? 1u : (uint32_t)RT_TRACE_LIMIT - left;
            if (kind == 1u) c_limit++; else c_hits++;
            if (kind == 2u) c_border += 1u + ((r.nk & kFreshInvalid) ? 1u : 0u);
            else if (!LRZ && ps_border(pr_vox(r))) c_border++;
        }
    };
    auto first_step = [&](PSlot& r, bool en) {
        en = en && ps_running(r.nk);
        uint32_t st = 0;
        if (en) st = lookup(ps_vox(r));
        p_advance<true, 1, LOGR, LRZ>(r, st, en, swz, f.lr[0], f.lr[1], f.lr[2]);
    };

    auto stack_at = [&](uint32_t c, uint32_t j) -> uint32_t {
        if constexpr (STK == 0) {
            return s_stack[c][j][threadIdx.x];
        } else if constexpr (STK == 2) {
            if (j < 3u) return s_stack[c][j][threadIdx.x];
            return a.stack[((size_t)c * stack_levels + j) * a.nthreads + gtid];
        } else {
            return a.stack[((size_t)c * stack_levels + j) * a.nthreads + gtid];
        }
    };
    auto stack_put = [&](uint32_t c, uint32_t j, uint32_t m) {
        if (LDS_ROWS && (STK == 0 || j < 3u)) s_stack[c][j][threadIdx.x] = m;
        else a.stack[((size_t)c * stack_levels + j) * a.nthreads + gtid] = m;
    };

    constexpr uint32_t PP_SNAN = 1u << 19, PP_FNAN = 1u << 18;
    auto pass = [&]() {
        const bool endA = !lm_lane(rSA | rFA), endB = !lm_lane(rSB | rFB);
        const bool workA = endA && !(exhausted && (PA.st >> 20) == 0u), workB = endB && !(exhausted && (PB.st >> 20) == 0u);
        const bool act = workA || workB, useB = !workA && workB;
        const uint32_t c = useB ? 1u : 0u;
        const uint32_t Fnk = useB ? FB.nk : FA.nk;
        const float Fpx = useB ? FB.px : FA.px, Fpy = useB ? FB.py : FA.py, Fpz = useB ? FB.pz : FA.pz;
        const float Fdx = useB ? FB.ndx : FA.ndx, Fdy = useB ? FB.ndy : FA.ndy, Fdz = useB ? FB.ndz : FA.ndz;
        const uint32_t Fvox = useB ? pr_vox(FB) : pr_vox(FA);
        const lanemask useBm = __ballot(useB);
        const uint32_t Faxis = lm_lane((zFB & useBm) | (zFA & ~useBm)) ? 2u : (lm_lane((xyFB & useBm) | (xyFA & ~useBm)) ? 0u : 1u);
        const bool Sair = useB ? pr_outside<LOGR, LRZ>(SB.px, SB.py, SB.pz, f.lr[0], f.lr[1], f.lr[2])
                               : pr_outside<LOGR, LRZ>(SA.px, SA.py, SA.pz, f.lr[0], f.lr[1], f.lr[2]);
        const bool Fair = pr_outside<LOGR, LRZ>(Fpx, Fpy, Fpz, f.lr[0], f.lr[1], f.lr[2]);
        uint32_t Pst = useB ? PB.st : PA.st, Pitem = useB ? PB.item : PA.item, Pent = useB ? PB.ent : PA.ent;

        const uint32_t level = Pst >> 20;
        const bool mine = act && level != 0u;
        const bool fin = mine && (Fair || (Pst & PP_FINAL) != 0u);
        const bool cont = mine && !fin;
        if (COUNT) {
            d_passf++; d_plf += (uint32_t)__popcll(__ballot(mine));
            if (mine) { if (useB) { tally(FB); tally(SB); } else { tally(FA); tally(SA); } }
        }
        bool getnew = false;
        uint32_t nsb = 0, nw = 0;
        if (!exhausted) {
            const bool wantme = act && (level == 0u || fin);
            const uint64_t want = __ballot(wantme);
            const uint32_t nwant = (uint32_t)__popcll(want);
            if (nwant) {
                if (chunk_next >= chunk_end) {
// ... 100 lines not shown
            hx = Faxis == 0u ? hx + offv : hx; hy = Faxis == 1u ? hy + offv : hy; hz = Faxis == 2u ? hz + offv : hz;
            stack_put(c, level - 1u, (hit && !(!LRZ && ps_border(Fvox))) ? matv : 0u);
            Pst = sunbits | (Pst & (PP_SNAN | PP_FNAN)) | (level + 1u) << 20 | (level + 1u == D ? PP_FINAL : 0u);
            sfx = hx; sfy = hy; sfz = hz; snormal = nrm;
            start = true;
        }
        if (getnew) {
            sfx = ox; sfy = oy; sfz = oz;
            snormal = info >> 28;
            Pitem = nsb * nwork + nw;
            Pent = nse | 7u << 16;
            Pst = 1u << 20 | (D == 1u ? PP_FINAL : 0u);
            start = true;
        }

        const uint32_t se = Pent & 0xFFFFu;
        const bool newface = start && snormal != Pent >> 16;
        const uint32_t di = newface ? 4u * ((snormal << 16) | se) : 0u;
        const uint32_t si = getnew ? 2u * se : 0u;
        const float4 d2 = a.dif_lut[di + 1u], dl = a.dif_lut[di + 2u];
        const float4 sd = a.sun_lut[si], sl = a.sun_lut[si + 1u];
        if (COUNT && start) { c_noise++; c_shadow++; c_dif++; }
        int ix, iy, iz;
        const bool ok = wrap_texel(v3(sfx, sfy, sfz), (float)R, &ix, &iy, &iz);
        const uint32_t tx = s_swz[ix], ty = s_swz[kTabWords + iy], tz = s_swz[2u * kTabWords + iz];
        if (newface) {
            Pent = se | snormal << 16;
            Pst = (Pst & ~PP_FNAN) | ((d2.x != d2.x || d2.y != d2.y || d2.z != d2.z) ? PP_FNAN : 0u);
        }
        if (getnew) Pst |= (sd.x != sd.x || sd.y != sd.y || sd.z != sd.z) ? PP_SNAN : 0u;
        bool runS = start && !((Pst & PP_SNAN) || !ok), runF = start && !((Pst & PP_FNAN) || !ok);
        const uint32_t nk0 = (uint32_t)RT_TRACE_LIMIT | ((COUNT && !ok) ? kFreshInvalid : 0u);
        const bool outside = start && ok && pr_outside<LOGR, LRZ>(sfx, sfy, sfz, f.lr[0], f.lr[1], f.lr[2]);
        const bool below = LRZ && outside && (sfx + half < 0.0f || sfy + half < 0.0f || sfz + half < 0.0f);

        float Spx = sfx, Spy = sfy, Spz = sfz, Tpx = sfx, Tpy = sfy, Tpz = sfz;
        uint32_t Ssx = tx, Ssy = ty, Ssz = tz, Tsx = tx, Tsy = ty, Tsz = tz, nkS = nk0, nkF = nk0;
        bool Tz = true, Txy = false;
        if (__builtin_expect(__ballot(below) != 0ull, 0)) {
            PSlot TS, TF;
            TS.px = sfx; TS.py = sfy; TS.pz = sfz; TS.sx = tx; TS.sy = ty; TS.sz = tz; TS.axis = 2u;
            TS.nk = runS ? (uint32_t)RT_TRACE_LIMIT : (K_DEAD | K_END);
            TF = TS; TF.nk = runF ? (uint32_t)RT_TRACE_LIMIT : (K_DEAD | K_END);
            TS.ndx = getnew ? -sd.x : (useB ? SB.ndx : SA.ndx); TS.ndy = getnew ? -sd.y : (useB ? SB.ndy : SA.ndy);
            TS.ndz = getnew ? -sd.z : (useB ? SB.ndz : SA.ndz);
            TS.lx = getnew ? sl.x : (useB ? SB.lx : SA.lx); TS.ly = getnew ? sl.y : (useB ? SB.ly : SA.ly); TS.lz = getnew ? sl.z : (useB ? SB.lz : SA.lz);
            TF.ndx = newface ? -d2.x : Fdx; TF.ndy = newface ? -d2.y : Fdy; TF.ndz = newface ? -d2.z : Fdz;
            TF.lx = newface ? dl.x : (useB ? FB.lx : FA.lx); TF.ly = newface ? dl.y : (useB ? FB.ly : FA.ly); TF.lz = newface ? dl.z : (useB ? FB.lz : FA.lz);
            first_step(TS, below); first_step(TF, below);
            if (below) {
                Spx = TS.px; Spy = TS.py; Spz = TS.pz; Ssx = TS.sx; Ssy = TS.sy; Ssz = TS.sz;
                Tpx = TF.px; Tpy = TF.py; Tpz = TF.pz; Tsx = TF.sx; Tsy = TF.sy; Tsz = TF.sz;
                if (runS) { runS = ps_running(TS.nk); nkS = TS.nk & 0xFFFFu; }
                if (runF) { runF = ps_running(TF.nk); nkF = TF.nk & 0xFFFFu; Tz = TF.axis == 2u; Txy = TF.axis == 0u; }
            }
        }
        if (__builtin_expect(__ballot(outside) != 0ull, 0)) {
            uint32_t st0 = 1u;
            if (outside) st0 = lookup(tx | ty | tz);
            const float qnan = __builtin_nanf("");
            if (outside && (nkS & 0xFFFFu) == (uint32_t)RT_TRACE_LIMIT && !(runS && st0 != 0u)) { Spx = Spy = Spz = qnan; runS = false; }
            if (outside && (nkF & 0xFFFFu) == (uint32_t)RT_TRACE_LIMIT && !(runF && st0 != 0u)) { Tpx = Tpy = Tpz = qnan; runF = false; }
        }

        if (useB) { PB.st = Pst; PB.item = Pitem; PB.ent = Pent; } else { PA.st = Pst; PA.item = Pitem; PA.ent = Pent; }
        const bool startA = start && !useB, startB = start && useB;
        if (startA) {
            SA.px = Spx; SA.py = Spy; SA.pz = Spz; SA.sx = Ssx; SA.sy = Ssy; SA.sz = Ssz; SA.nk = nkS;
            FA.px = Tpx; FA.py = Tpy; FA.pz = Tpz; FA.sx = Tsx; FA.sy = Tsy; FA.sz = Tsz; FA.nk = nkF;
        }
        if (startB) {
            SB.px = Spx; SB.py = Spy; SB.pz = Spz; SB.sx = Ssx; SB.sy = Ssy; SB.sz = Ssz; SB.nk = nkS;
            FB.px = Tpx; FB.py = Tpy; FB.pz = Tpz; FB.sx = Tsx; FB.sy = Tsy; FB.sz = Tsz; FB.nk = nkF;
        }
        {
            const lanemask sA = __ballot(startA), sB = __ballot(startB), mS = __ballot(runS), mF = __ballot(runF), mz = __ballot(Tz), mxy = __ballot(Txy);
            rSA = (rSA & ~sA) | (mS & sA); rFA = (rFA & ~sA) | (mF & sA); zFA = (zFA & ~sA) | (mz & sA); xyFA = (xyFA & ~sA) | (mxy & sA);
            rSB = (rSB & ~sB) | (mS & sB); rFB = (rFB & ~sB) | (mF & sB); zFB = (zFB & ~sB) | (mz & sB); xyFB = (xyFB & ~sB) | (mxy & sB);
        }
        if (newface && !useB) { FA.ndx = -d2.x; FA.ndy = -d2.y; FA.ndz = -d2.z; FA.lx = dl.x; FA.ly = dl.y; FA.lz = dl.z; }
        if (newface && useB) { FB.ndx = -d2.x; FB.ndy = -d2.y; FB.ndz = -d2.z; FB.lx = dl.x; FB.ly = dl.y; FB.lz = dl.z; }
        if (getnew && !useB) { SA.ndx = -sd.x; SA.ndy = -sd.y; SA.ndz = -sd.z; SA.lx = sl.x; SA.ly = sl.y; SA.lz = sl.z; }
        if (getnew && useB) { SB.ndx = -sd.x; SB.ndy = -sd.y; SB.ndz = -sd.z; SB.lx = sl.x; SB.ly = sl.y; SB.lz = sl.z; }
    };

#ifdef RT_DIAG_STEP_TIMES
    unsigned long long t_lds = 0, t_mem = 0, t_alu = 0, t_steps = 0, t_bytes = 0;
#endif
    auto step_all = [&](auto shadow_tag, auto careful_tag) {
        constexpr bool SHADOW = decltype(shadow_tag)::value, CAREFUL = decltype(careful_tag)::value;
#ifdef RT_DIAG_STEP_TIMES
        const bool timed = exhausted;
        unsigned long long tq0 = 0, tq1 = 0, tq2 = 0;
        if (timed) { asm volatile("s_waitcnt vmcnt(0) lgkmcnt(0)" ::: "memory"); tq0 = clock64(); }
#endif
        const uint32_t v1 = pr_vox(FA), v3_ = pr_vox(FB);
        uint32_t n1, n3, h1, h3;
        ps_nibble_of<LOGR, LRZ>(v1, &n1, &h1); ps_nibble_of<LOGR, LRZ>(v3_, &n3, &h3);
        uint32_t v0 = 0, v2 = 0, n0 = 0, n2 = 0, h0 = 0, h2 = 0, w0 = 0, w2 = 0;
        if (SHADOW) {
            v0 = pr_vox(SA); v2 = pr_vox(SB);
            ps_nibble_of<LOGR, LRZ>(v0, &n0, &h0); ps_nibble_of<LOGR, LRZ>(v2, &n2, &h2);
            w0 = s_nib[n0]; w2 = s_nib[n2];
        }
        const uint32_t w1 = s_nib[n1], w3 = s_nib[n3];
        uint32_t t1 = __builtin_amdgcn_ubfe(w1, h1, 4u), t3 = __builtin_amdgcn_ubfe(w3, h3, 4u);
        if (!LRZ) {
            t1 |= (uint32_t)((int32_t)v1 >> 31) & 15u; t3 |= (uint32_t)((int32_t)v3_ >> 31) & 15u;
        }
#ifdef RT_DIAG_STEP_TIMES
        if (timed) { asm volatile("s_waitcnt lgkmcnt(0)" ::: "memory"); tq1 = clock64(); }
#endif
        const lanemask m1 = rFA & __ballot(t1 == kNibMixed), m3 = rFB & __ballot(t3 == kNibMixed);
        const bool g1 = lm_lane(m1), g3 = lm_lane(m3);
        uint32_t t0 = 0, t2 = 0, b0 = 0, b2 = 0;
        bool g0 = false, g2 = false;
        lanemask m0 = 0, m2 = 0;
        if (SHADOW) {
            t0 = __builtin_amdgcn_ubfe(w0, h0, 4u); t2 = __builtin_amdgcn_ubfe(w2, h2, 4u);
            if (!LRZ) { t0 |= (uint32_t)((int32_t)v0 >> 31) & 15u; t2 |= (uint32_t)((int32_t)v2 >> 31) & 15u; }
            m0 = rSA & __ballot(t0 == kNibMixed); m2 = rSB & __ballot(t2 == kNibMixed);
            g0 = lm_lane(m0); g2 = lm_lane(m2);
        }
        if (COUNT) {
            d_fetch += (uint32_t)__popcll(rFA) + (uint32_t)__popcll(rFB) + (SHADOW ? (uint32_t)__popcll(rSA) + (uint32_t)__popcll(rSB) : 0u);
            d_fetch_cube += (uint32_t)__popcll(m1) + (uint32_t)__popcll(m3) + (uint32_t)__popcll(m0) + (uint32_t)__popcll(m2);
        }
        if constexpr (LOGR > 8 && RT_PATHS_BRICK_MAP != 0) {
            uint32_t u0 = 0, u2 = 0;
            if (SHADOW) u0 = __builtin_amdgcn_raw_buffer_load_b8(brick_rsrc, g0 ? v0 >> 7 : 0xFFFFFFFFu, 0, 0);
            uint32_t u1 = __builtin_amdgcn_raw_buffer_load_b8(brick_rsrc, g1 ? v1 >> 7 : 0xFFFFFFFFu, 0, 0);
            if (SHADOW) u2 = __builtin_amdgcn_raw_buffer_load_b8(brick_rsrc, g2 ? v2 >> 7 : 0xFFFFFFFFu, 0, 0);
            uint32_t u3 = __builtin_amdgcn_raw_buffer_load_b8(brick_rsrc, g3 ? v3_ >> 7 : 0xFFFFFFFFu, 0, 0);
            u1 = __builtin_amdgcn_ubfe(u1, (v1 >> 4) & 4u, 4u); u3 = __builtin_amdgcn_ubfe(u3, (v3_ >> 4) & 4u, 4u);
            const lanemask n1 = m1 & __ballot(u1 == kNibMixed), n3 = m3 & __ballot(u3 == kNibMixed);
            const bool k1 = lm_lane(n1), k3 = lm_lane(n3);
            bool k0 = false, k2 = false;
            lanemask n0 = 0, n2 = 0;
            if (SHADOW) {
                u0 = __builtin_amdgcn_ubfe(u0, (v0 >> 4) & 4u, 4u); u2 = __builtin_amdgcn_ubfe(u2, (v2 >> 4) & 4u, 4u);
                n0 = m0 & __ballot(u0 == kNibMixed); n2 = m2 & __ballot(u2 == kNibMixed);
                k0 = lm_lane(n0); k2 = lm_lane(n2);
                b0 = __builtin_amdgcn_raw_buffer_load_b8(mine_rsrc, k0 ? v0 : 0xFFFFFFFFu, 0, 0);
            }
            if (COUNT) d_fetch_brick += (uint32_t)__popcll(n1) + (uint32_t)__popcll(n3) + (uint32_t)__popcll(n0) + (uint32_t)__popcll(n2);
            const uint32_t b1 = __builtin_amdgcn_raw_buffer_load_b8(mine_rsrc, k1 ? v1 : 0xFFFFFFFFu, 0, 0);
            if (SHADOW) b2 = __builtin_amdgcn_raw_buffer_load_b8(mine_rsrc, k2 ? v2 : 0xFFFFFFFFu, 0, 0);
            const uint32_t b3 = __builtin_amdgcn_raw_buffer_load_b8(mine_rsrc, k3 ? v3_ : 0xFFFFFFFFu, 0, 0);
            t1 = g1 ? (k1 ? b1 : u1) : t1; t3 = g3 ? (k3 ? b3 : u3) : t3;
            if (SHADOW) { t0 = g0 ? (k0 ? b0 : u0) : t0; t2 = g2 ? (k2 ? b2 : u2) : t2; }
        } else {
            if (COUNT) d_fetch_brick += (uint32_t)__popcll(m1) + (uint32_t)__popcll(m3) + (uint32_t)__popcll(m0) + (uint32_t)__popcll(m2);
            if (SHADOW) b0 = __builtin_amdgcn_raw_buffer_load_b8(mine_rsrc, g0 ? v0 : 0xFFFFFFFFu, 0, 0);
            const uint32_t b1 = __builtin_amdgcn_raw_buffer_load_b8(mine_rsrc, g1 ? v1 : 0xFFFFFFFFu, 0, 0);
            if (SHADOW) b2 = __builtin_amdgcn_raw_buffer_load_b8(mine_rsrc, g2 ? v2 : 0xFFFFFFFFu, 0, 0);
            const uint32_t b3 = __builtin_amdgcn_raw_buffer_load_b8(mine_rsrc, g3 ? v3_ : 0xFFFFFFFFu, 0, 0);
            t1 = g1 ? b1 : t1; t3 = g3 ? b3 : t3;
            if (SHADOW) { t0 = g0 ? b0 : t0; t2 = g2 ? b2 : t2; }
        }
#ifdef RT_DIAG_STEP_TIMES
        if (timed) {
            asm volatile("s_waitcnt vmcnt(0)" ::: "memory"); tq2 = clock64();
            t_bytes += (uint32_t)__popcll(__ballot(g1)) + (uint32_t)__popcll(__ballot(g3)) + (uint32_t)__popcll(__ballot(g0)) + (uint32_t)__popcll(__ballot(g2));
        }
#endif
        if (SHADOW) p_step<false, LOGR, LRZ, CAREFUL>(SA, rSA, nul, nul2, t0, swz, f.lr[0], f.lr[1], f.lr[2]);
        p_step<true, LOGR, LRZ, CAREFUL>(FA, rFA, zFA, xyFA, t1, swz, f.lr[0], f.lr[1], f.lr[2]);
        if (SHADOW) p_step<false, LOGR, LRZ, CAREFUL>(SB, rSB, nul, nul2, t2, swz, f.lr[0], f.lr[1], f.lr[2]);
        p_step<true, LOGR, LRZ, CAREFUL>(FB, rFB, zFB, xyFB, t3, swz, f.lr[0], f.lr[1], f.lr[2]);
#ifdef RT_DIAG_STEP_TIMES
        if (timed) {
            asm volatile("s_waitcnt lgkmcnt(0)" ::: "memory");
            const unsigned long long tq3 = clock64();
            t_lds += tq1 - tq0; t_mem += tq2 - tq1; t_alu += tq3 - tq2; t_steps++;
        }
#endif
    };
    constexpr uint32_t kLimitMargin = 16u * RT_PATHS_STEPS_PER_CHECK + 4u;
    auto near_limit = [&]() -> lanemask {
        return (rSA & __ballot((SA.nk & 0xFFFFu) < kLimitMargin)) | (rFA & __ballot((FA.nk & 0xFFFFu) < kLimitMargin)) |
               (rSB & __ballot((SB.nk & 0xFFFFu) < kLimitMargin)) | (rFB & __ballot((FB.nk & 0xFFFFu) < kLimitMargin));
    };

    for (;;) {
        uint64_t park;
        for (;;) {
            const uint64_t eA = ~(rSA | rFA), eB = ~(rSB | rFB);
            uint64_t idleA = 0ull, idleB = 0ull;
            if (exhausted) { idleA = __ballot((PA.st >> 20) == 0u); idleB = __ballot((PB.st >> 20) == 0u); }
            park = (eA & ~idleA) | (eB & ~idleB);
            if ((uint32_t)__popcll(park) >= (exhausted ? (uint32_t)RT_PATHS_DRAIN_PARK : threshold) || (eA & eB) == ~0ull) break;
            if (COUNT) { d_iters++; d_live += (uint32_t)__popcll(~eA) + (uint32_t)__popcll(~eB); }
            if (__builtin_expect((looks++ & 15u) == 0u, 0)) {
                while (__builtin_expect(near_limit() != 0ull, 0)) step_all(std::true_type{}, std::true_type{});
            }
#pragma unroll
            for (int rep = 0; rep < RT_PATHS_STEPS_PER_CHECK; rep++) {
                if (LOGR != 8 || (RT_PATHS_SHADOW_REPS >> rep & 1) != 0) step_all(std::true_type{}, std::false_type{});
                else step_all(std::false_type{}, std::false_type{});
            }
        }
        if (park == 0ull) break;
#ifdef RT_DIAG_WAVE_TIMES
        if (exhausted && !t_exh) t_exh = wall_clock64();
#endif
        __builtin_amdgcn_s_setprio(1);
        pass();
        __builtin_amdgcn_s_setprio(0);
    }
    if (COUNT) {
        DevCounters* cn = a.counters;
        const unsigned long long rays = c_shadow + c_dif;
        wave_add(&cn->rays, rays); wave_add(&cn->rays_shadow, c_shadow);
        wave_add(&cn->rays_diffuse, c_dif); wave_add(&cn->iterations, c_iter); wave_add(&cn->minefield_fetches, rays + c_iter);
        wave_add(&cn->hits, c_hits); wave_add(&cn->material_fetches, c_hits); wave_add(&cn->sky_exits, c_sky);
        wave_add(&cn->limit_exits, c_limit); wave_add(&cn->border_fetches, c_border); wave_add(&cn->noise_fetches, c_noise);
        if (lane == 0) {
#ifndef RT_DIAG_WAVE_TIMES
            atomicAdd(&cn->dbg_loop_iters, d_iters); atomicAdd(&cn->dbg_f_lanes, d_live);
            atomicAdd(&cn->dbg_passes, d_passf); atomicAdd(&cn->dbg_pass_lanes, d_plf);
#ifdef RT_DIAG_STEP_TIMES
            (void)d_fetch; (void)d_fetch_cube; (void)d_fetch_brick;
            atomicAdd(&cn->dbg_s_execs, t_lds); atomicAdd(&cn->dbg_s_lanes, t_mem); atomicAdd(&cn->dbg_sky_lanes, t_alu);
            atomicAdd(&cn->dbg_f_execs, t_steps); atomicAdd(&cn->dbg_loop_iters, t_bytes);
#else
            atomicAdd(&cn->dbg_s_execs, d_fetch); atomicAdd(&cn->dbg_s_lanes, d_fetch_cube); atomicAdd(&cn->dbg_sky_lanes, d_fetch_brick);
#endif
#else
            (void)d_iters; (void)d_live; (void)d_passf; (void)d_plf; (void)d_fetch; (void)d_fetch_cube; (void)d_fetch_brick;
            const unsigned long long t1 = wall_clock64();
            atomicAdd(&cn->dbg_s_execs, t1 - t_wave0); atomicMax(&cn->dbg_f_execs, t1); atomicMax(&cn->dbg_sky_lanes, ~t_wave0);
            atomicAdd(&cn->dbg_s_lanes, t_exh ? t1 - t_exh : 0ull);
            atomicMax(&cn->dbg_loop_iters, t_exh ? ~t_exh : 0ull);
            atomicAdd(&cn->dbg_passes, 1ull);
            atomicAdd(&cn->dbg_pass_lanes, t1 & 0xFFFFFFFFFFull);
            atomicAdd(&cn->dbg_f_lanes, (t_exh ? t_exh : t1) & 0xFFFFFFFFFFull);
            if (STK == 0) {
                unsigned long long* rec = reinterpret_cast<unsigned long long*>(a.stack) + (size_t)(gtid >> 6) * 4u;
                rec[0] = t_wave0; rec[1] = t_exh; rec[2] = t1; rec[3] = blockIdx.x;
            }
#endif
        }
    }
}

bool launch_paths_direct_ok(const Frame& f) { return f.depth <= 4 && f.logr == 8; }

hipError_t launch_paths(const Scene& sc, const Frame& f, const Planes& pl, const PersistArgs& a, bool count, int nworkgroups,
                        hipStream_t st) {
    if (f.logr < 8 || f.logr > 10) return hipErrorInvalidValue;
    const dim3 grid(nworkgroups), block(1024);
    const bool lds_stack = f.depth <= 4 && f.logr == 8;
    const bool lrz = f.lr_zero != 0;
#define RT_LAUNCH_PATHS(C, S, L, Z) hipLaunchKernelGGL((k_paths<C, S, L, Z>), grid, block, 0, st, sc, f, pl, a)
#define RT_LAUNCH_PATHS_CZ(S, L) do { if (count) { if (lrz) RT_LAUNCH_PATHS(true, S, L, true); else RT_LAUNCH_PATHS(true, S, L, false); } \
                                      else { if (lrz) RT_LAUNCH_PATHS(false, S, L, true); else RT_LAUNCH_PATHS(false, S, L, false); } } while (0)
    if (f.logr == 8) {
        if (lds_stack) RT_LAUNCH_PATHS_CZ(0, 8); else if (f.depth <= 8) RT_LAUNCH_PATHS_CZ(2, 8); else RT_LAUNCH_PATHS_CZ(1, 8);
    } else if (f.logr == 9) {
        RT_LAUNCH_PATHS_CZ(1, 9);
    } else {
        RT_LAUNCH_PATHS_CZ(1, 10);
    }
#undef RT_LAUNCH_PATHS_CZ
#undef RT_LAUNCH_PATHS
    return hipGetLastError();
}

}
```

### raytrace_amd/csrc/rt_pslot.hpp

```cpp
#pragma once
#include <hip/hip_runtime.h>

#include "rt_device.hpp"

namespace rtd {
namespace pslot {

enum : uint32_t { K_END = 1u << 16, K_AIR = 1u << 17, K_DEAD = 1u << 18 };
constexpr uint32_t kFreshInvalid = 1u << 24;
template <int LOGR> constexpr uint32_t swz_bytes() { return 8u << LOGR; }
constexpr uint32_t kSwzBytes = swz_bytes<8>();
constexpr uint32_t kSwzBorder = 0x80000000u;

typedef __attribute__((address_space(3))) uint32_t lds_u32;

struct PSlot {
    float px, py, pz, ndx, ndy, ndz, lx, ly, lz;
    uint32_t sx, sy, sz, nk, axis;
};
__device__ __forceinline__ uint32_t ps_vox(const PSlot& r) { return r.sx | r.sy | r.sz; }
__device__ __forceinline__ bool ps_border(uint32_t vox) { return (vox & kSwzBorder) != 0u; }
template <int LOGR, bool LRZ = true>
__device__ __forceinline__ void ps_nibble_of(uint32_t vox, uint32_t* byte, uint32_t* shift) {
    if (LOGR == 8) { *byte = LRZ ? vox >> 7 : (vox >> 7) & 0x1FFFFu; *shift = (vox >> 4) & 4u; return; }
    constexpr int LB = LOGR - 2, SUB = LOGR - 8;
    const uint32_t c = ((vox >> (6 + SUB)) & 63u) | ((vox >> (LB + SUB)) & (63u << 6)) | ((vox >> (2 * LB + SUB - 6)) & (63u << 12));
    *byte = c >> 1; *shift = (c & 1u) << 2;
}
__device__ __forceinline__ uint32_t ps_axis_of_code(uint32_t code) { return (code & 2u) ? ((code & 1u) ? 0u : 1u) : 2u; }
__device__ __forceinline__ bool ps_running(uint32_t nk) { return nk - 1u < (uint32_t)RT_TRACE_LIMIT; }

constexpr uint32_t PP_FINAL = K_AIR;
struct PPath { uint32_t st, item, ent; };

__device__ __forceinline__ float f_bits(uint32_t u) { return __builtin_bit_cast(float, u); }
__device__ __forceinline__ uint32_t u_bits(float f) { return __builtin_bit_cast(uint32_t, f); }

template <bool GENERIC_Q, int AXIS, int LOGR = 8, bool LRZ = true>
__device__ __forceinline__ void p_advance(PSlot& r, uint32_t st, bool enable, uint32_t swz, float lrx = 0.0f, float lry = 0.0f, float lrz = 0.0f) {
    constexpr float half = (float)(1 << (LOGR - 1));
    const uint32_t nk = r.nk;
    const bool go = enable && ps_running(nk) && st != 0u;
    const uint32_t sb = (st << 23) + (126u << 23);
    const float sz = f_bits(sb), is = f_bits(0x7F000000u - sb);
    const float ux = r.px + half, uy = r.py + half, uz = r.pz + half;
    float qx, qy, qz;
    if (GENERIC_Q) {
        qx = r.ndx < 0.0f ? -ux : ux; qy = r.ndy < 0.0f ? -uy : uy; qz = r.ndz < 0.0f ? -uz : uz;
    } else if (!LRZ) {
        qx = f_bits(u_bits(ux) ^ (u_bits(r.ndx) & 0x80000000u));
        qy = f_bits(u_bits(uy) ^ (u_bits(r.ndy) & 0x80000000u));
        qz = f_bits(u_bits(uz) ^ (u_bits(r.ndz) & 0x80000000u));
    } else {
        qx = f_bits((u_bits(ux) & 0x7FFFFFFFu) | (u_bits(r.ndx) & 0x80000000u));
        qy = f_bits((u_bits(uy) & 0x7FFFFFFFu) | (u_bits(r.ndy) & 0x80000000u));
        qz = f_bits((u_bits(uz) & 0x7FFFFFFFu) | (u_bits(r.ndz) & 0x80000000u));
    }
    const float mx = __builtin_fmaf(-sz, rtm_floor(qx * is), qx);
    const float my = __builtin_fmaf(-sz, rtm_floor(qy * is), qy);
    const float mz = __builtin_fmaf(-sz, rtm_floor(qz * is), qz);
    const float tx = (0.0001f + mx) * r.lx, ty = (0.0001f + my) * r.ly, tz = (0.0001f + mz) * r.lz;
    const float t = __builtin_fminf(__builtin_fminf(tx, ty), tz);
    if (AXIS == 1) {
        const uint32_t ax = tz == t ? 2u : (tx < ty ? 0u : 1u);
        r.axis = go ? ax : r.axis;
    }
    if (AXIS == 2) {
        const uint32_t notz = (u_bits(t) - u_bits(tz)) >> 31;
        const uint32_t xlt = (u_bits(tx) - u_bits(ty)) >> 31;
        const uint32_t code = notz + notz + xlt;
        r.axis = go ? code : r.axis;
    }
    const float te = go ? t : 0.0f;
    r.px = __builtin_fmaf(-r.ndx, te, r.px); r.py = __builtin_fmaf(-r.ndy, te, r.py); r.pz = __builtin_fmaf(-r.ndz, te, r.pz);
    const bool sky = LRZ ? __builtin_fmaxf(__builtin_fmaxf(rtm_abs(r.px), rtm_abs(r.py)), rtm_abs(r.pz)) >= half
                         : __builtin_fmaxf(__builtin_fmaxf(rtm_abs(r.px - lrx), rtm_abs(r.py - lry)), rtm_abs(r.pz - lrz)) >= half;
    const uint32_t moved = nk + (sky ? (K_AIR | K_END) - 1u : 0xFFFFFFFFu);
    r.nk = go ? moved : (nk | K_END);
    constexpr float four_half = 4.0f * half;
    constexpr uint32_t kMask = swz_bytes<LOGR>() - 4u, kTab = swz_bytes<LOGR>();
    float x4 = __builtin_fmaf(r.px, 4.0f, four_half), y4 = __builtin_fmaf(r.py, 4.0f, four_half), z4 = __builtin_fmaf(r.pz, 4.0f, four_half);
    if (!LRZ) {
        constexpr float four_r = 8.0f * half, inv_four_r = 1.0f / four_r;
        x4 = __builtin_fmaf(-four_r, rtm_floor(x4 * inv_four_r), x4);
        y4 = __builtin_fmaf(-four_r, rtm_floor(y4 * inv_four_r), y4);
        z4 = __builtin_fmaf(-four_r, rtm_floor(z4 * inv_four_r), z4);
    }
    const uint32_t ix = (uint32_t)(int)x4, iy = (uint32_t)(int)y4, iz = (uint32_t)(int)z4;
    r.sx = *(lds_u32*)(uintptr_t)((ix & kMask) | swz);
    r.sy = *(lds_u32*)(uintptr_t)((iy & kMask) | (swz + kTab));
    r.sz = *(lds_u32*)(uintptr_t)((iz & kMask) | (swz + 2u * kTab));
}

struct PRay {
    float px, py, pz, ndx, ndy, ndz, lx, ly, lz;
    uint32_t sx, sy, sz, nk;
};
typedef uint64_t lanemask;
__device__ __forceinline__ bool lm_lane(lanemask m) { return __builtin_amdgcn_inverse_ballot_w64(m); }
__device__ __forceinline__ uint32_t pr_vox(const PRay& r) { return r.sx | r.sy | r.sz; }
template <int LOGR, bool LRZ>
__device__ __forceinline__ bool pr_outside(float px, float py, float pz, float lrx, float lry, float lrz) {
    constexpr float half = (float)(1 << (LOGR - 1));
    return LRZ ? __builtin_fmaxf(__builtin_fmaxf(rtm_abs(px), rtm_abs(py)), rtm_abs(pz)) >= half
               : __builtin_fmaxf(__builtin_fmaxf(rtm_abs(px - lrx), rtm_abs(py - lry)), rtm_abs(pz - lrz)) >= half;
}

template <bool DIFFUSE, int LOGR, bool LRZ, bool CAREFUL>
__device__ __forceinline__ void p_step(PRay& r, lanemask& run, lanemask& az, lanemask& axy, uint32_t st, uint32_t swz, float lrx, float lry, float lrz) {
    constexpr float half = (float)(1 << (LOGR - 1));
    if (CAREFUL) asm volatile("; careful step" ::: "memory");
    lanemask go = run & __ballot(st != 0u);
    if (CAREFUL) go &= __ballot((r.nk & 0xFFFFu) != 0u);
    uint32_t sb;
    asm("v_lshl_add_u32 %0, %1, 23, 0.5" : "=v"(sb) : "v"(st));
    const float sz = f_bits(sb), is = f_bits(0x7F000000u - sb);
    const float ux = r.px + half, uy = r.py + half, uz = r.pz + half;
    float qx, qy, qz;
    if (!LRZ) {
        qx = f_bits(u_bits(ux) ^ (u_bits(r.ndx) & 0x80000000u));
        qy = f_bits(u_bits(uy) ^ (u_bits(r.ndy) & 0x80000000u));
        qz = f_bits(u_bits(uz) ^ (u_bits(r.ndz) & 0x80000000u));
    } else {
        qx = f_bits((u_bits(ux) & 0x7FFFFFFFu) | (u_bits(r.ndx) & 0x80000000u));
        qy = f_bits((u_bits(uy) & 0x7FFFFFFFu) | (u_bits(r.ndy) & 0x80000000u));
        qz = f_bits((u_bits(uz) & 0x7FFFFFFFu) | (u_bits(r.ndz) & 0x80000000u));
    }
    const float mx = __builtin_fmaf(-sz, rtm_floor(qx * is), qx);
    const float my = __builtin_fmaf(-sz, rtm_floor(qy * is), qy);
    const float mz = __builtin_fmaf(-sz, rtm_floor(qz * is), qz);
    const float tx = (0.0001f + mx) * r.lx, ty = (0.0001f + my) * r.ly, tz = (0.0001f + mz) * r.lz;
    const float t = __builtin_fminf(__builtin_fminf(tx, ty), tz);
    if (DIFFUSE) { az = (go & __ballot(tz == t)) | (az & ~go); axy = (go & __ballot(tx < ty)) | (axy & ~go); }
#ifdef RT_PSTEP_TE_SELECT
    {
        const bool gol = lm_lane(go);
        const float te = gol ? t : 0.0f;
        r.px = __builtin_fmaf(-r.ndx, te, r.px); r.py = __builtin_fmaf(-r.ndy, te, r.py); r.pz = __builtin_fmaf(-r.ndz, te, r.pz);
        r.nk -= gol ? 1u : 0u;
    }
#else
    {
        lanemask saved;
        asm("s_and_saveexec_b64 %[sv], %[go]\n\t"
            "v_fma_f32 %[px], -%[dx], %[t], %[px]\n\t"
            "v_fma_f32 %[py], -%[dy], %[t], %[py]\n\t"
            "v_fma_f32 %[pz], -%[dz], %[t], %[pz]\n\t"
            "v_add_u32_e32 %[nk], -1, %[nk]\n\t"
            "s_mov_b64 exec, %[sv]"
            : [px] "+v"(r.px), [py] "+v"(r.py), [pz] "+v"(r.pz), [nk] "+v"(r.nk), [sv] "=&s"(saved)
            : [go] "s"(go), [t] "v"(t), [dx] "v"(r.ndx), [dy] "v"(r.ndy), [dz] "v"(r.ndz)
            : "scc");
    }
#endif
    run = go & ~__ballot(pr_outside<LOGR, LRZ>(r.px, r.py, r.pz, lrx, lry, lrz));
    constexpr float four_half = 4.0f * half;
    constexpr uint32_t kMask = swz_bytes<LOGR>() - 4u, kTab = swz_bytes<LOGR>();
    float x4 = __builtin_fmaf(r.px, 4.0f, four_half), y4 = __builtin_fmaf(r.py, 4.0f, four_half), z4 = __builtin_fmaf(r.pz, 4.0f, four_half);
    if (!LRZ) {
        constexpr float four_r = 8.0f * half, inv_four_r = 1.0f / four_r;
        x4 = __builtin_fmaf(-four_r, rtm_floor(x4 * inv_four_r), x4);
        y4 = __builtin_fmaf(-four_r, rtm_floor(y4 * inv_four_r), y4);
        z4 = __builtin_fmaf(-four_r, rtm_floor(z4 * inv_four_r), z4);
    }
    const uint32_t ix = (uint32_t)(int)x4, iy = (uint32_t)(int)y4, iz = (uint32_t)(int)z4;
    r.sx = *(lds_u32*)(uintptr_t)((ix & kMask) | swz);
    r.sy = *(lds_u32*)(uintptr_t)((iy & kMask) | (swz + kTab));
    r.sz = *(lds_u32*)(uintptr_t)((iz & kMask) | (swz + 2u * kTab));
    if (CAREFUL) asm volatile("; careful step end" ::: "memory");
}

}
}
```

### raytrace_amd/csrc/rt_world.hip

```cpp
#include <hip/hip_runtime.h>

#include "rt_kernels.hpp"
#include "rt_world.hpp"

namespace rtd {

__global__ __launch_bounds__(256) void k_flatten_voxels(const uint8_t* __restrict__ mine_lin,
                                                        const uint32_t* __restrict__ mat_lin,
                                                        uint8_t* __restrict__ mine_sw, uint32_t* __restrict__ mat_sw,
                                                        uint32_t* __restrict__ bad_value_flag, int logr) {
    const uint32_t i = blockIdx.x * 256u + threadIdx.x;
    const int lb = logr - 2;
    const uint32_t bmask = (1u << lb) - 1u;
    uint32_t brick = i >> 6, l = i & 63u;
    uint32_t ix = ((brick & bmask) << 2) | (l & 3u);
    uint32_t iy = (((brick >> lb) & bmask) << 2) | ((l >> 2) & 3u);
    uint32_t iz = ((brick >> (2 * lb)) << 2) | (l >> 4);
    size_t src = (((((size_t)iz << logr) + iy) << logr)) + ix;
    uint8_t v = mine_lin[src];
    if (v > kMaxStepValue) atomicOr(bad_value_flag, 1u);
    mine_sw[i] = v;
    mat_sw[i] = mat_lin[src];
}

__global__ __launch_bounds__(256) void k_flatten_slab(const uint8_t* __restrict__ mine_slab, const uint32_t* __restrict__ mat_slab,
                                                      uint8_t* __restrict__ mine_sw, uint32_t* __restrict__ mat_sw,
                                                      int logr, int axis, int offset) {
    const uint32_t i = blockIdx.x * 256u + threadIdx.x;
    const int lb = logr - 2;
    const uint32_t bmask = (1u << lb) - 1u;
    const uint32_t l = i & 63u, sb = i >> 6;
    uint32_t bc[3];
    uint32_t rest = sb;
    for (int a = 0; a < 3; a++) {
        if (a == axis) { bc[a] = (uint32_t)(offset >> 2) + (rest & 3u); rest >>= 2; }
        else { bc[a] = rest & bmask; rest >>= lb; }
    }
    const uint32_t ix = (bc[0] << 2) | (l & 3u), iy = (bc[1] << 2) | ((l >> 2) & 3u), iz = (bc[2] << 2) | (l >> 4);
    const uint32_t R = 1u << logr;
    const uint32_t sx = axis == 0 ? ix - (uint32_t)offset : ix, sy = axis == 1 ? iy - (uint32_t)offset : iy,
                   sz = axis == 2 ? iz - (uint32_t)offset : iz;
    const uint32_t ex = axis == 0 ? (uint32_t)RT_SLICE_SIZE : R, ey = axis == 1 ? (uint32_t)RT_SLICE_SIZE : R;
    const size_t src = ((size_t)sz * ey + sy) * ex + sx;
    const size_t dst = ((size_t)brick_index(bc[0], bc[1], bc[2], lb) << 6) | l;
    mine_sw[dst] = mine_slab[src];
    mat_sw[dst] = mat_slab[src];
}

__global__ __launch_bounds__(256) void k_build_maps(const uint8_t* __restrict__ mine_sw, uint32_t* __restrict__ coarse,
                                                    uint32_t* __restrict__ brick_words, int logr, MapBoxes box) {
    const uint32_t t = blockIdx.x * 256u + threadIdx.x;
    const uint32_t ncw = box.cwn.x * box.cwn.y * box.cwn.z, nbw = brick_words ? box.bwn.x * box.bwn.y * box.bwn.z : 0u;
    const int lb = logr - 2;
    if (t < ncw) {
        const uint32_t wx = box.cw0.x + t % box.cwn.x, cy = box.cw0.y + (t / box.cwn.x) % box.cwn.y, cz = box.cw0.z + t / (box.cwn.x * box.cwn.y);
        const uint32_t w = (cz << 9) | (cy << 3) | wx;
        coarse[w] = coarse_word(mine_sw, w, logr);
    } else if (t - ncw < nbw) {
        const uint32_t u = t - ncw;
        const uint32_t wx = box.bw0.x + u % box.bwn.x, by = box.bw0.y + (u / box.bwn.x) % box.bwn.y, bz = box.bw0.z + u / (box.bwn.x * box.bwn.y);
        const uint32_t w = brick_index(8u * wx, by, bz, lb) >> 3;
        brick_words[w] = brick_word(mine_sw, w);
    }
}

__device__ uint32_t nibble_of_cube(const uint8_t* mine_sw, int x0, int y0, int z0, int e, int lb) {
    const uint8_t v = mine_sw[swizzled_index(x0, y0, z0, lb)];
    for (int z = z0; z < z0 + e; z++)
        for (int y = y0; y < y0 + e; y++)
            for (int x = x0; x < x0 + e; x++)
                if (mine_sw[swizzled_index(x, y, z, lb)] != v) return kNibMixed;
    return v < kNibMixed ? v : kNibMixed;
}

__global__ __launch_bounds__(256) void k_check_maps(const uint8_t* __restrict__ mine_sw, const uint32_t* __restrict__ coarse,
                                                    const uint32_t* __restrict__ brick_words, uint32_t nbrick_words, int logr,
                                                    unsigned long long* __restrict__ mismatches) {
    const uint32_t t = blockIdx.x * 256u + threadIdx.x;
    const int lb = logr - 2, e = 1 << (logr - 6), nb = 1 << lb;
    bool differs = false;
    if (t < (uint32_t)kCoarseWords) {
        uint32_t word = 0;
        for (int b = 0; b < 8; b++) {
            const int c = (int)t * 8 + b;
            word |= nibble_of_cube(mine_sw, (c & 63) * e, ((c >> 6) & 63) * e, (c >> 12) * e, e, lb) << (4 * b);
        }
        differs = word != coarse[t];
    } else if (t - (uint32_t)kCoarseWords < nbrick_words) {
        const uint32_t u = t - (uint32_t)kCoarseWords;
        uint32_t word = 0;
        for (int b = 0; b < 8; b++) {
            const int k = (int)u * 8 + b;
            word |= nibble_of_cube(mine_sw, (k & (nb - 1)) * 4, ((k >> lb) & (nb - 1)) * 4, (k >> (2 * lb)) * 4, 4, lb) << (4 * b);
        }
        differs = word != brick_words[u];
    }
    const uint64_t m = __ballot(differs);
    if ((threadIdx.x & 63u) == 0u && m) atomicAdd(mismatches, (unsigned long long)__popcll(m));
}

__global__ __launch_bounds__(256) void k_read_box(const uint8_t* __restrict__ mine_sw, const uint32_t* __restrict__ mat_sw, int logr,
                                                  int x0, int y0, int z0, int ex, int ey, uint64_t n, uint32_t* __restrict__ mat_out,
                                                  uint8_t* __restrict__ mine_out) {
    const uint64_t i = (uint64_t)blockIdx.x * 256u + threadIdx.x;
    if (i >= n) return;
    const int x = x0 + (int)(i % (uint64_t)ex), y = y0 + (int)((i / (uint64_t)ex) % (uint64_t)ey), z = z0 + (int)(i / ((uint64_t)ex * ey));
    const uint32_t s = swizzled_index(x, y, z, logr - 2);
    if (mat_out) mat_out[i] = mat_sw[s];
    if (mine_out) mine_out[i] = mine_sw[s];
}

MapBoxes map_boxes_region(int logr) {
    const uint32_t nb = 1u << (logr - 2);
    return MapBoxes{make_uint3(0, 0, 0), make_uint3(8, 64, 64), make_uint3(0, 0, 0), make_uint3(nb / 8u, nb, nb)};
}

MapBoxes map_boxes_slab(int logr, int axis, int texel_offset) {
    MapBoxes b = map_boxes_region(logr);
    const uint32_t off = (uint32_t)texel_offset, e = (1u << logr) / 64u;
    const uint32_t c0 = off / e, c1 = (off + RT_SLICE_SIZE - 1u) / e;
    const uint32_t b0 = off / 4u;
    if (axis == 0) { b.cw0.x = c0 / 8u; b.cwn.x = c1 / 8u - b.cw0.x + 1u; b.bw0.x = b0 / 8u; b.bwn.x = (b0 + 3u) / 8u - b.bw0.x + 1u; }
    else if (axis == 1) { b.cw0.y = c0; b.cwn.y = c1 - c0 + 1u; b.bw0.y = b0; b.bwn.y = 4u; }
    else { b.cw0.z = c0; b.cwn.z = c1 - c0 + 1u; b.bw0.z = b0; b.bwn.z = 4u; }
    return b;
}

hipError_t launch_build_maps(const uint8_t* mine_sw, uint32_t* coarse, uint32_t* brick, int logr, const MapBoxes& b, hipStream_t st) {
    uint32_t* bmap = logr > 8 ? brick : nullptr;
    const uint32_t n = b.cwn.x * b.cwn.y * b.cwn.z + (bmap ? b.bwn.x * b.bwn.y * b.bwn.z : 0u);
    hipLaunchKernelGGL(k_build_maps, dim3((n + 255u) / 256u), dim3(256), 0, st, mine_sw, coarse, bmap, logr, b);
    return hipGetLastError();
}

hipError_t launch_flatten(const uint8_t* mine_lin, const uint32_t* mat_lin, uint8_t* mine_sw, uint32_t* mat_sw,
                          uint32_t* coarse, uint32_t* brick, uint32_t* bad_flag, int logr, hipStream_t st) {
    hipLaunchKernelGGL(k_flatten_voxels, dim3((1u << (3 * logr)) / 256u), dim3(256), 0, st, mine_lin, mat_lin, mine_sw, mat_sw,
                       bad_flag, logr);
    return launch_build_maps(mine_sw, coarse, brick, logr, map_boxes_region(logr), st);
}

hipError_t launch_flatten_slab(const uint8_t* mine_slab, const uint32_t* mat_slab, uint8_t* mine_sw, uint32_t* mat_sw, uint32_t* coarse,
                               uint32_t* brick, int logr, int axis, int offset, hipStream_t st) {
    const uint32_t R = 1u << logr;
    hipLaunchKernelGGL(k_flatten_slab, dim3(RT_SLICE_SIZE * R * R / 256u), dim3(256), 0, st, mine_slab, mat_slab, mine_sw, mat_sw,
                       logr, axis, offset);
    return launch_build_maps(mine_sw, coarse, brick, logr, map_boxes_slab(logr, axis, offset), st);
}

hipError_t launch_check_maps(const uint8_t* mine_sw, const uint32_t* coarse, const uint32_t* brick, int logr,
                             unsigned long long* mismatches, hipStream_t st) {
    const uint32_t nbw = (logr > 8 && brick) ? (1u << (3 * (logr - 2))) / 8u : 0u;
    const uint32_t n = (uint32_t)kCoarseWords + nbw;
    hipLaunchKernelGGL(k_check_maps, dim3((n + 255u) / 256u), dim3(256), 0, st, mine_sw, coarse, nbw ? brick : nullptr, nbw, logr,
                       mismatches);
    return hipGetLastError();
}

hipError_t launch_read_box(const uint8_t* mine_sw, const uint32_t* mat_sw, int logr, int x0, int y0, int z0, int ex, int ey, int nz,
                           uint32_t* mat_out, uint8_t* mine_out, hipStream_t st) {
    const uint64_t n = (uint64_t)ex * (uint64_t)ey * (uint64_t)nz;
    if (n == 0) return hipSuccess;
    hipLaunchKernelGGL(k_read_box, dim3((unsigned)((n + 255u) / 256u)), dim3(256), 0, st, mine_sw, mat_sw, logr, x0, y0, z0, ex, ey, n,
                       mat_out, mine_out);
    return hipGetLastError();
}

}
```

### raytrace_amd/render.py

```python
import ctypes as C
import math

import numpy as np

from . import _lib
from .abi import (BUFFER_FORMATS, BUFFER_NAMES, MAX_DRAW_BOXES, MAX_DRAW_STAMPS, MAX_POINT_LIGHTS, RT_BUF_COUNT, RT_BUF_FINAL_BGRA8, RT_KERNEL_DEFAULT, RT_SHAPE_BOX, RT_SHAPE_SPHERE,
                  RT_SWEEP_BLOCKED, RT_SWEEP_FREE, RT_WHERE_ALL, RtBoxSweep, RtConfig, RtCounters, RtDenoiseParams, RtDrawBox, RtDrawStamp, RtInfo, RtLightProbe,
                  RtPointLight, RtProbeLight, RtRayHit, RtShapeEdit, RtStampPlace, RtSweepHit, RtTiming, RtUniforms, RtVoxelEdit)


class RtError(RuntimeError):
    def __init__(self, code, message):
        super().__init__("rt error %d: %s" % (code, message))
        self.code = code


def make_config(width, height, spp=1, depth=2, device=0, tile_rank=0, tile_world=1, kernel=RT_KERNEL_DEFAULT, flags=0,
                region=256, history_cap=0, edit_radius=0, stream_history=0):
    cfg = RtConfig()
    cfg.struct_size = C.sizeof(RtConfig)
    cfg.width, cfg.height, cfg.region = int(width), int(height), int(region)
    cfg.spp, cfg.depth, cfg.device = int(spp), int(depth), int(device)
    cfg.tile_rank, cfg.tile_world = int(tile_rank), int(tile_world)
    cfg.kernel, cfg.flags = int(kernel), int(flags)
# ... 411 lines not shown
        return self._lib.rt_gbuffer_ptr(self._h)

    def gbuffer_bytes(self):
        return int(self._lib.rt_gbuffer_bytes(self._h))

    def gbuffer_offset(self, buffer_id):
        return int(self._lib.rt_gbuffer_offset(self._h, int(buffer_id)))

    def untile_gbuffer(self, gathered_dev_ptr, world, frame_dev_ptrs):
        arr = (C.c_void_p * 6)(*[C.c_void_p(p) if p else None for p in frame_dev_ptrs])
        self._check(self._lib.rt_untile_gbuffer(self._h, C.c_void_p(gathered_dev_ptr), int(world), arr))

    def comm_init_rank(self, unique_id):
        comm = C.c_void_p()
        buf = (C.c_char * len(unique_id)).from_buffer_copy(bytes(unique_id))
        self._check(self._lib.rt_comm_init_rank(self._h, buf, len(unique_id), C.byref(comm)))
        return comm.value

    def gather_gbuffer(self, comm, root, frame_dev_ptrs=None, overlapped=False):
        arr = (C.c_void_p * 6)(*[C.c_void_p(p) if p else None for p in frame_dev_ptrs]) if frame_dev_ptrs else None
        self._check(self._lib.rt_gather_gbuffer(self._h, C.c_void_p(comm) if comm else None, int(root), arr, 1 if overlapped else 0))

    def selftest(self, which=1):
        out = C.c_uint64(0)
        self._check(self._lib.rt_selftest(self._h, int(which), C.byref(out)))
        return int(out.value)

    def frame_ptr(self, buffer_id):
        return self._lib.rt_frame_ptr(self._h, int(buffer_id))

    def frame_readback(self, buffer_id):
        dt, ch = BUFFER_FORMATS[buffer_id]
        W, H = self.cfg.width, self.cfg.height
        out = np.empty((H, W, ch) if ch > 1 else (H, W), dtype=dt)
        self._check(self._lib.rt_frame_readback(self._h, int(buffer_id), _p(out), out.nbytes))
        return out

    def denoise(self, faithful=True):
        self._check(self._lib.rt_denoise(self._h, 1 if faithful else 0))

    def finalize(self):
        self._check(self._lib.rt_finalize(self._h))

    def denoise_planes(self, lighting_ptr, depth_ptr, normal_ptr, faithful=True):
        self._check(self._lib.rt_denoise_planes(self._h, C.c_void_p(lighting_ptr), C.c_void_p(depth_ptr), C.c_void_p(normal_ptr),
                                                1 if faithful else 0))

    def denoise_history(self, params=None, faithful=True):
        if params is None:
            params = denoise_params(faithful=faithful, **HISTORY_DENOISE_PRESET)
        self._check(self._lib.rt_denoise_history(self._h, C.byref(params)))

    def denoise_planes_counted(self, lighting_ptr, depth_ptr, normal_ptr, counts_ptr, params):
        self._check(self._lib.rt_denoise_planes_counted(self._h, C.c_void_p(lighting_ptr), C.c_void_p(depth_ptr), C.c_void_p(normal_ptr),
                                                        C.c_void_p(counts_ptr), C.byref(params)))

    def finalize_planes(self, albedo_ptr, emission_ptr, fog_ptr, lighting_ptr, depth_ptr, out_ptr):
        self._check(self._lib.rt_finalize_planes(self._h, C.c_void_p(albedo_ptr), C.c_void_p(emission_ptr), C.c_void_p(fog_ptr),
                                                 C.c_void_p(lighting_ptr), C.c_void_p(depth_ptr), C.c_void_p(out_ptr)))

    def kernel_in_use(self):
        return int(self._lib.rt_kernel_in_use(self._h))

    def counters(self):
        cn = RtCounters()
        self._check(self._lib.rt_get_counters(self._h, C.byref(cn)))
        return cn

    def reset_counters(self):
        self._check(self._lib.rt_reset_counters(self._h))

    def reset_accumulation(self):
        self._check(self._lib.rt_reset_accumulation(self._h))

    def accumulation(self):
        frames, samples = C.c_uint32(0), C.c_uint32(0)
        self._check(self._lib.rt_get_accumulation(self._h, C.byref(frames), C.byref(samples)))
        return int(frames.value), int(samples.value)

    def read_history(self):
        out = np.empty((self.cfg.height, self.cfg.width), dtype=np.uint32)
        self._check(self._lib.rt_read_history(self._h, _p(out), out.nbytes))
        return out

    def edit_boxes_pending(self):
        boxes, over = C.c_uint32(0), C.c_uint32(0)
        self._check(self._lib.rt_edit_boxes_pending(self._h, C.byref(boxes), C.byref(over)))
        return int(boxes.value), bool(over.value)

    def slabs_pending(self):
        slabs, over = C.c_uint32(0), C.c_uint32(0)
        self._check(self._lib.rt_slabs_pending(self._h, C.byref(slabs), C.byref(over)))
        return int(slabs.value), bool(over.value)

    def read_slab_boxes(self):
        out = np.zeros((8, 2, 3), dtype=np.float32)
        n = C.c_uint32(0)
        self._check(self._lib.rt_read_slab_boxes(self._h, _p(out), C.byref(n)))
        return out[:int(n.value)].copy()

    def info(self):
        i = RtInfo()
        i.struct_size = C.sizeof(RtInfo)
        self._check(self._lib.rt_get_info(self._h, C.byref(i)))
        return i

    def timing(self):
        t = RtTiming()
        self._check(self._lib.rt_get_timing(self._h, C.byref(t)))
        return t

    def gather_timing(self):
        ms, n = C.c_float(0.0), C.c_uint32(0)
        self._check(self._lib.rt_get_gather_timing(self._h, C.byref(ms), C.byref(n)))
        return float(ms.value), int(n.value)



def compute_triple_euler_vector(heading, pitch):
    f = (C.c_float * 3)()
    u = (C.c_float * 3)()
    r = (C.c_float * 3)()
    _lib.host().rth_compute_triple_euler_vector(float(heading), float(pitch), f, u, r)
    return (np.array(f[:], dtype=np.float32), np.array(u[:], dtype=np.float32), np.array(r[:], dtype=np.float32))


class Camera:

    def __init__(self, game):
        self._game = game

    def _get(self):
        o = (C.c_float * 3)()
        h = C.c_float()
        p = C.c_float()
        _lib.host().rth_game_get_camera(self._game._h, o, C.byref(h), C.byref(p))
        return [o[0], o[1], o[2]], h.value, p.value

    @property
    def origin(self):
        return tuple(self._get()[0])

    @property
    def heading(self):
        return self._get()[1]

    @property
    def pitch(self):
        return self._get()[2]

    def set(self, origin=None, heading=None, pitch=None):
        o, h, p = self._get()
        if origin is not None:
            o = list(origin)
        if heading is not None:
            h = heading
        if pitch is not None:
            p = pitch
        _lib.host().rth_game_set_camera(self._game._h, (C.c_float * 3)(*o), float(h), float(p))


class Game:

    def __init__(self, args=()):
        argv = [b"raytrace"] + [str(a).encode() for a in args]
        arr = (C.c_char_p * len(argv))(*argv)
# ... 442 lines not shown
```

Before: 54770.

## Add open-sky coarse map allowing larger empty-space steps for steep downward rays

Builds a per-region 'open map' with three kernels: find the top ground height per coarse column, dilate it with a distance cone, and re-encode each coarse nibble with an extra bit marking cells that lie safely above the terrain cone. The depth 5..8 paths kernel at region 256 reads this map instead of the plain coarse map. Steep downward rays that do not graze grid lines keep the larger step value in open cells, and all other rays mask the bit off. The aim is fewer traversal steps through empty sky. The cost is a rebuild whenever the world changes, extra memory, and added per-ray mask work and register pressure in the hot kernel.

```diff
diff --git a/include/rt_abi.h b/include/rt_abi.h
--- a/include/rt_abi.h
+++ b/include/rt_abi.h
@@ -359,6 +359,8 @@
 int rt_slabs_pending(RtContext* ctx, uint32_t* slabs, uint32_t* overflowed);
 int rt_read_slab_boxes(RtContext* ctx, float* boxes, uint32_t* count);
 
+int rt_read_open_map(RtContext* ctx, uint32_t* words, size_t bytes);
+
 int rt_get_counters(RtContext* ctx, RtCounters* out);
 int rt_reset_counters(RtContext* ctx);
 int rt_get_timing(RtContext* ctx, RtTiming* out);
diff --git a/raytrace_amd/_lib.py b/raytrace_amd/_lib.py
--- a/raytrace_amd/_lib.py
+++ b/raytrace_amd/_lib.py
@@ -21,7 +21,7 @@
     "rt_denoise_history", "rt_denoise_planes_counted", "rt_sweep_boxes", "rt_sweep_boxes_async",
     "rt_edit_shapes", "rt_draw_boxes", "rt_draw_boxes_async", "rt_add_lights", "rt_add_lights_async",
     "rt_stamp_create", "rt_stamp_capture", "rt_stamp_info", "rt_stamp_read", "rt_stamp_destroy", "rt_edit_stamps",
-    "rt_draw_stamps", "rt_draw_stamps_async", "rt_shadow_entities", "rt_shadow_entities_async",
+    "rt_draw_stamps", "rt_draw_stamps_async", "rt_shadow_entities", "rt_shadow_entities_async", "rt_read_open_map",
 )
 
 _amd = None
@@ -127,6 +127,9 @@
             getattr(lib, name).restype = C.c_int
         lib.rt_read_box.argtypes = [P, C.c_int, C.c_int, C.c_int, C.c_int, C.c_int, C.c_int, P, P]
         lib.rt_read_box.restype = C.c_int
+        if hasattr(lib, "rt_read_open_map"):
+            lib.rt_read_open_map.argtypes = [P, P, C.c_size_t]
+            lib.rt_read_open_map.restype = C.c_int
         lib.rt_trace_rays.argtypes = [P, P, C.c_uint32, C.POINTER(C.c_int32), P]
         lib.rt_trace_rays.restype = C.c_int
         lib.rt_trace_rays_async.argtypes = [P, P, C.c_uint32, C.POINTER(C.c_int32), P]
diff --git a/raytrace_amd/csrc/api/api_context.hip b/raytrace_amd/csrc/api/api_context.hip
--- a/raytrace_amd/csrc/api/api_context.hip
+++ b/raytrace_amd/csrc/api/api_context.hip
@@ -56,6 +56,7 @@
 
 void invalidate_prepass(RtContext* c) {
     for (FrameSlot& fs : c->slots) fs.prepass_valid = false;
+    c->open_stale = true;
 }
 
 void plane_written(RtContext* c, const void* ptr) {
@@ -195,6 +196,14 @@
         RT_HIP(c, dev_alloc(c, &c->d_slab_masks, (size_t)rtd::kSlabSlots * rtd::kSlabSlotWords));
         RT_HIP(c, dev_alloc(c, &c->d_slab_boxes, 1));
         RT_HIP(c, hipMemset(c->d_slab_boxes, 0, sizeof(rtd::SlabBoxes)));
+    }
+    int paths_open = 1;
+    env_int("RT_PATHS_OPEN", 0, 1, &paths_open);
+    rtd::Frame fopen{};
+    fopen.depth = cfg.depth; fopen.logr = c->logr; fopen.lr_zero = 1;
+    if (paths_open && rtd::launch_paths_uses_open_map(fopen, (cfg.flags & RT_FLAG_COUNTERS) != 0)) {
+        RT_HIP(c, dev_alloc(c, &c->d_open, (size_t)rtd::kCoarseWords));
+        RT_HIP(c, dev_alloc(c, &c->d_open_scratch, rtd::kOpenScratchWords));
     }
     RT_HIP(c, rtd::launch_sphere_lut(c->sphere_lut, c->own_stream));
     RT_HIP(c, rtd::launch_dif_lut(c->sphere_lut, c->dif_lut, c->own_stream));
diff --git a/raytrace_amd/csrc/api/api_frame.hip b/raytrace_amd/csrc/api/api_frame.hip
--- a/raytrace_amd/csrc/api/api_frame.hip
+++ b/raytrace_amd/csrc/api/api_frame.hip
@@ -197,6 +197,21 @@
     return e;
 }
 
+hipError_t frame_open_map(RtContext* c, PersistFrame& p) {
+    const uint32_t spp = (uint32_t)c->cfg.spp, B = c->persist_batch;
+    if (!c->d_open || !c->open_stale || c->route.frame || !p.cache || c->cfg.depth < 1 || !c->route.on_paths(spp < B ? spp : B) ||
+        !rtd::launch_paths_uses_open_map(p.f, p.count))
+        return hipSuccess;
+    hipError_t e = p.nl == 2 ? join_lanes_into(c, p.st0) : hipSuccess;
+    {
+        LaunchTimer t(c, 1, p.st0);
+        if (e == hipSuccess) e = rtd::launch_build_open_map(c->d_mine_sw, c->d_coarse, c->d_open, c->d_open_scratch, p.st0);
+    }
+    if (e == hipSuccess && p.nl == 2) e = fence_lanes_after(c, p.st0);
+    c->open_stale = e != hipSuccess;
+    return e;
+}
+
 hipError_t frame_prepass(RtContext* c, PersistFrame& p) {
     FrameSlot& fs = *p.fs;
     const bool prepass_clears = c->primary_version == 2 && c->npix_pad != 0;
@@ -278,7 +293,7 @@
         pa.pl_stream = stream_st ? 1u : 0u;
         if (e == hipSuccess) {
             LaunchTimer t(c, 0, st);
-            e = to_paths ? rtd::launch_paths(scene_of(c), p.f, p.pl, pa, p.count, c->num_cus, st)
+            e = to_paths ? rtd::launch_paths(scene_of(c), p.f, p.pl, pa, p.count, c->num_cus, st, c->open_stale ? nullptr : c->d_open)
                          : rtd::launch_persist(scene_of(c), p.f, p.pl, pa, p.count, p.cache, 1, c->num_cus, st);
         }
         if (e == hipSuccess && !r.direct) {
@@ -353,6 +368,7 @@
     hipError_t e = frame_begin(c, p, u, frame_events);
     if (e == hipSuccess && p.cache && !c->route.frame && !p.reuse) e = frame_prepass(c, p);
     if (e == hipSuccess) e = frame_tables(c, p);
+    if (e == hipSuccess) e = frame_open_map(c, p);
     if (e == hipSuccess && c->route.frame) e = frame_one_launch(c, p);
     else if (e == hipSuccess && (!p.cache || c->cfg.depth >= 1)) e = frame_path_batches(c, p);
     if (e == hipSuccess && p.accum) e = frame_accumulate_tail(c, p);
diff --git a/raytrace_amd/csrc/api/api_world.hip b/raytrace_amd/csrc/api/api_world.hip
--- a/raytrace_amd/csrc/api/api_world.hip
+++ b/raytrace_amd/csrc/api/api_world.hip
@@ -440,6 +440,23 @@
     return RT_OK;
 }
 
+int rt_read_open_map(RtContext* ctx, uint32_t* words, size_t bytes) {
+    if (!ctx) return RT_ERR_INVALID_ARG;
+    if (!ctx->d_open) return fail(ctx, RT_ERR_INVALID_ARG, "rt_read_open_map: the context keeps no open map (region above 256, counters, depth outside 5..8, a baseline kernel, or RT_PATHS_OPEN=0)");
+    if (!words || bytes != (size_t)rtd::kCoarseWords * sizeof(uint32_t)) return fail(ctx, RT_ERR_INVALID_ARG, "rt_read_open_map: null destination or size mismatch");
+    if (!ctx->world_resident) return fail(ctx, RT_ERR_NOT_READY, "rt_read_open_map: no region uploaded");
+    RT_HIP(ctx, hipSetDevice(ctx->device));
+    RT_HIP(ctx, sync_lanes(ctx));
+    if (ctx->open_stale) {
+        RT_HIP(ctx, rtd::launch_build_open_map(ctx->d_mine_sw, ctx->d_coarse, ctx->d_open, ctx->d_open_scratch, ctx->stream));
+        RT_HIP(ctx, fence_lanes_after(ctx, ctx->stream));
+        ctx->open_stale = false;
+    }
+    RT_HIP(ctx, hipMemcpyAsync(words, ctx->d_open, bytes, hipMemcpyDeviceToHost, ctx->stream));
+    RT_HIP(ctx, hipStreamSynchronize(ctx->stream));
+    return RT_OK;
+}
+
 int rt_read_box(RtContext* ctx, int x0, int y0, int z0, int ex, int ey, int ez, uint32_t* materials, uint8_t* minefield) {
     if (!ctx) return RT_ERR_INVALID_ARG;
     const int R = ctx->region;
diff --git a/raytrace_amd/csrc/api/rt_context.hpp b/raytrace_amd/csrc/api/rt_context.hpp
--- a/raytrace_amd/csrc/api/rt_context.hpp
+++ b/raytrace_amd/csrc/api/rt_context.hpp
@@ -157,6 +157,9 @@
     uint8_t* d_mine_sw = nullptr; uint32_t* d_mat_sw = nullptr;
     uint32_t* d_coarse = nullptr; uint32_t* d_noise = nullptr; uint32_t* d_flag = nullptr;
     uint32_t* d_brick = nullptr;
+    uint32_t* d_open = nullptr;
+    int32_t* d_open_scratch = nullptr;
+    bool open_stale = true;
     hipStream_t upload_stream = nullptr;
     rta::StagingSet slab_sets[2], edit_sets[2];
     uint64_t slabs = 0, edit_batches = 0;
diff --git a/raytrace_amd/csrc/rt_device.hpp b/raytrace_amd/csrc/rt_device.hpp
--- a/raytrace_amd/csrc/rt_device.hpp
+++ b/raytrace_amd/csrc/rt_device.hpp
@@ -12,6 +12,13 @@
 constexpr int kCoarseWords = kCoarseCount / 8;
 constexpr uint32_t kNibMixed = 15;
 constexpr uint32_t kMaxStepValue = 30;
+
+constexpr int kOpenSlope = 1;
+constexpr int kOpenMarginVoxels = 1;
+constexpr float kOpenSteepDz = 0.7072f;
+constexpr float kOpenGridClearance = 0.01f;
+constexpr uint32_t kOpenBit = 8;
+constexpr int kOpenNoGround = -(1 << 20);
 
 __device__ __forceinline__ uint32_t swizzled_index(int ix, int iy, int iz, int lb) {
     const uint32_t brick = ((uint32_t)(iz >> 2) << (2 * lb)) | ((uint32_t)(iy >> 2) << lb) | (uint32_t)(ix >> 2);
diff --git a/raytrace_amd/csrc/rt_kernels.hpp b/raytrace_amd/csrc/rt_kernels.hpp
--- a/raytrace_amd/csrc/rt_kernels.hpp
+++ b/raytrace_amd/csrc/rt_kernels.hpp
@@ -115,8 +115,9 @@
                           int version , int nworkgroups, hipStream_t st);
 
 bool launch_paths_direct_ok(const Frame& f);
+bool launch_paths_uses_open_map(const Frame& f, bool count);
 hipError_t launch_paths(const Scene& sc, const Frame& f, const Planes& pl, const PersistArgs& a, bool count, int nworkgroups,
-                        hipStream_t st);
+                        hipStream_t st, const uint32_t* open_map = nullptr);
 
 struct MapBoxes { uint3 cw0, cwn, bw0, bwn; };
 MapBoxes map_boxes_region(int logr);
@@ -129,6 +130,8 @@
                                uint32_t* brick, int logr, int axis, int offset, hipStream_t st);
 hipError_t launch_check_maps(const uint8_t* mine_sw, const uint32_t* coarse, const uint32_t* brick, int logr,
                              unsigned long long* mismatches, hipStream_t st);
+constexpr size_t kOpenScratchWords = 2 * (size_t)kCoarsePerAxis * kCoarsePerAxis;
+hipError_t launch_build_open_map(const uint8_t* mine_sw, const uint32_t* coarse, uint32_t* open_map, int32_t* scratch, hipStream_t st);
 hipError_t launch_read_box(const uint8_t* mine_sw, const uint32_t* mat_sw, int logr, int x0, int y0, int z0, int ex, int ey, int nz,
                            uint32_t* mat_out, uint8_t* mine_out, hipStream_t st);
 hipError_t launch_rebuild_chunks(uint8_t* mine_sw, uint32_t* mat_sw, const uint32_t* chunks, const uint32_t* offs, const uint2* recs,
diff --git a/raytrace_amd/csrc/rt_paths.hip b/raytrace_amd/csrc/rt_paths.hip
--- a/raytrace_amd/csrc/rt_paths.hip
+++ b/raytrace_amd/csrc/rt_paths.hip
@@ -22,9 +22,16 @@
 namespace rtd {
 using namespace pslot;
 
-template <bool COUNT, int STK, int LOGR, bool LRZ>
+#ifdef RT_DIAG_OPEN_COUNT
+constexpr bool kOpenCounts = true;
+#else
+constexpr bool kOpenCounts = false;
+#endif
+
+template <bool COUNT, int STK, int LOGR, bool LRZ, bool OPEN = false>
 __global__ __launch_bounds__(1024) void k_paths(Scene sc, Frame f, Planes pl, PersistArgs a) {
     static_assert(LOGR == 8 || STK == 1, "the larger regions' tables leave no LDS for the albedo stack");
+    static_assert(!OPEN || ((!COUNT || kOpenCounts) && LRZ && LOGR == 8 && STK == 2), "the open map serves non-counting lr = 0 launches of depth 5..8 at region 256");
     constexpr bool LDS_ROWS = STK == 0 || STK == 2;
     constexpr int R = 1 << LOGR, LB = LOGR - 2;
     constexpr uint32_t kTabWords = swz_bytes<LOGR>() / 4u;
@@ -93,6 +100,7 @@
         uint32_t nb, nsh;
         ps_nibble_of<LOGR, LRZ>(vox, &nb, &nsh);
         uint32_t st = (s_nib[nb] >> nsh) & 15u;
+        if (OPEN && st != kNibMixed) st &= kOpenBit - 1u;
         if (LOGR > 8 && RT_PATHS_BRICK_MAP != 0 && st == kNibMixed) st = (sc.brick[vox >> 7] >> ((vox >> 4) & 4u)) & 15u;
         if (st == kNibMixed) st = sc.mine[vox];
         return st;
@@ -359,6 +367,14 @@
         if (newface && useB) { FB.ndx = -d2.x; FB.ndy = -d2.y; FB.ndz = -d2.z; FB.lx = dl.x; FB.ly = dl.y; FB.lz = dl.z; }
         if (getnew && !useB) { SA.ndx = -sd.x; SA.ndy = -sd.y; SA.ndz = -sd.z; SA.lx = sl.x; SA.ly = sl.y; SA.lz = sl.z; }
         if (getnew && useB) { SB.ndx = -sd.x; SB.ndy = -sd.y; SB.ndz = -sd.z; SB.lx = sl.x; SB.ly = sl.y; SB.lz = sl.z; }
+        if (OPEN) {
+            const uint32_t plain = (kOpenBit - 1u) << kOpenMaskShift;
+            const float ux = useB ? SB.ndx : SA.ndx, uy = useB ? SB.ndy : SA.ndy, uz = useB ? SB.ndz : SA.ndz, ul = useB ? SB.lz : SA.lz;
+            const uint32_t mS = outside ? plain : open_step_mask<LOGR>(sfx, sfy, sfz, ux, uy, uz, ul);
+            const uint32_t mF = plain;
+            if (startA) { SA.nk |= mS; FA.nk |= mF; }
+            if (startB) { SB.nk |= mS; FB.nk |= mF; }
+        }
     };
 
 #ifdef RT_DIAG_STEP_TIMES
@@ -389,6 +405,7 @@
         if (timed) { asm volatile("s_waitcnt lgkmcnt(0)" ::: "memory"); tq1 = clock64(); }
 #endif
         const lanemask m1 = rFA & __ballot(t1 == kNibMixed), m3 = rFB & __ballot(t3 == kNibMixed);
+        if (OPEN) { t1 &= FA.nk >> kOpenMaskShift; t3 &= FB.nk >> kOpenMaskShift; }
         const bool g1 = lm_lane(m1), g3 = lm_lane(m3);
         uint32_t t0 = 0, t2 = 0, b0 = 0, b2 = 0;
         bool g0 = false, g2 = false;
@@ -397,6 +414,7 @@
             t0 = __builtin_amdgcn_ubfe(w0, h0, 4u); t2 = __builtin_amdgcn_ubfe(w2, h2, 4u);
             if (!LRZ) { t0 |= (uint32_t)((int32_t)v0 >> 31) & 15u; t2 |= (uint32_t)((int32_t)v2 >> 31) & 15u; }
             m0 = rSA & __ballot(t0 == kNibMixed); m2 = rSB & __ballot(t2 == kNibMixed);
+            if (OPEN) { t0 &= SA.nk >> kOpenMaskShift; t2 &= SB.nk >> kOpenMaskShift; }
             g0 = lm_lane(m0); g2 = lm_lane(m2);
         }
         if (COUNT) {
@@ -523,8 +541,10 @@
 
 bool launch_paths_direct_ok(const Frame& f) { return f.depth <= 4 && f.logr == 8; }
 
+bool launch_paths_uses_open_map(const Frame& f, bool count) { return (!count || kOpenCounts) && f.lr_zero != 0 && f.logr == 8 && f.depth > 4 && f.depth <= 8; }
+
 hipError_t launch_paths(const Scene& sc, const Frame& f, const Planes& pl, const PersistArgs& a, bool count, int nworkgroups,
-                        hipStream_t st) {
+                        hipStream_t st, const uint32_t* open_map) {
     if (f.logr < 8 || f.logr > 10) return hipErrorInvalidValue;
     const dim3 grid(nworkgroups), block(1024);
     const bool lds_stack = f.depth <= 4 && f.logr == 8;
@@ -532,7 +552,12 @@
 #define RT_LAUNCH_PATHS(C, S, L, Z) hipLaunchKernelGGL((k_paths<C, S, L, Z>), grid, block, 0, st, sc, f, pl, a)
 #define RT_LAUNCH_PATHS_CZ(S, L) do { if (count) { if (lrz) RT_LAUNCH_PATHS(true, S, L, true); else RT_LAUNCH_PATHS(true, S, L, false); } \
                                       else { if (lrz) RT_LAUNCH_PATHS(false, S, L, true); else RT_LAUNCH_PATHS(false, S, L, false); } } while (0)
-    if (f.logr == 8) {
+    if (open_map && launch_paths_uses_open_map(f, count)) {
+        Scene so = sc;
+        so.coarse = open_map;
+        if constexpr (kOpenCounts) { if (count) { hipLaunchKernelGGL((k_paths<true, 2, 8, true, kOpenCounts>), grid, block, 0, st, so, f, pl, a); return hipGetLastError(); } }
+        hipLaunchKernelGGL((k_paths<false, 2, 8, true, true>), grid, block, 0, st, so, f, pl, a);
+    } else if (f.logr == 8) {
         if (lds_stack) RT_LAUNCH_PATHS_CZ(0, 8); else if (f.depth <= 8) RT_LAUNCH_PATHS_CZ(2, 8); else RT_LAUNCH_PATHS_CZ(1, 8);
     } else if (f.logr == 9) {
         RT_LAUNCH_PATHS_CZ(1, 9);
diff --git a/raytrace_amd/csrc/rt_pslot.hpp b/raytrace_amd/csrc/rt_pslot.hpp
--- a/raytrace_amd/csrc/rt_pslot.hpp
+++ b/raytrace_amd/csrc/rt_pslot.hpp
@@ -96,6 +96,16 @@
     float px, py, pz, ndx, ndy, ndz, lx, ly, lz;
     uint32_t sx, sy, sz, nk;
 };
+constexpr uint32_t kOpenMaskShift = 16;
+template <int LOGR>
+__device__ __forceinline__ uint32_t open_step_mask(float ox, float oy, float oz, float ndx, float ndy, float ndz, float lz) {
+    constexpr float half = (float)(1 << (LOGR - 1));
+    const float t = (half - oz) * lz;
+    const float cx = __builtin_fmaf(-ndx, t, ox), cy = __builtin_fmaf(-ndy, t, oy);
+    const float gx = rtm_abs(cx - __builtin_rintf(cx)), gy = rtm_abs(cy - __builtin_rintf(cy));
+    const bool steep = ndz <= -kOpenSteepDz && gx >= kOpenGridClearance && gy >= kOpenGridClearance;
+    return (steep ? 15u : (kOpenBit - 1u)) << kOpenMaskShift;
+}
 typedef uint64_t lanemask;
 __device__ __forceinline__ bool lm_lane(lanemask m) { return __builtin_amdgcn_inverse_ballot_w64(m); }
 __device__ __forceinline__ uint32_t pr_vox(const PRay& r) { return r.sx | r.sy | r.sz; }
diff --git a/raytrace_amd/csrc/rt_world.hip b/raytrace_amd/csrc/rt_world.hip
--- a/raytrace_amd/csrc/rt_world.hip
+++ b/raytrace_amd/csrc/rt_world.hip
@@ -99,6 +99,73 @@
     if ((threadIdx.x & 63u) == 0u && m) atomicAdd(mismatches, (unsigned long long)__popcll(m));
 }
 
+__device__ __forceinline__ bool has_zero_byte(uint4 v) {
+    const uint32_t m = ((v.x - 0x01010101u) & ~v.x) | ((v.y - 0x01010101u) & ~v.y) | ((v.z - 0x01010101u) & ~v.z) | ((v.w - 0x01010101u) & ~v.w);
+    return (m & 0x80808080u) != 0u;
+}
+__global__ __launch_bounds__(256) void k_open_heights(const uint8_t* __restrict__ mine_sw, const uint32_t* __restrict__ coarse,
+                                                      int32_t* __restrict__ top) {
+    const uint32_t b = blockIdx.x * 256u + threadIdx.x;
+    int32_t t = kOpenNoGround;
+    for (int bz = kCoarsePerAxis - 1; bz >= 0 && t == kOpenNoGround; bz--) {
+        const uint32_t c = ((uint32_t)bz << 12) | b;
+        const uint32_t n = (coarse[c >> 3] >> (4u * (c & 7u))) & 15u;
+        if (n == 0u) t = 4 * bz + 4;
+        else if (n == kNibMixed) {
+            const Brick k = load_brick(mine_sw, c);
+            if (has_zero_byte(k.e)) t = 4 * bz + 4;
+            else if (has_zero_byte(k.d)) t = 4 * bz + 3;
+            else if (has_zero_byte(k.q)) t = 4 * bz + 2;
+            else if (has_zero_byte(k.a)) t = 4 * bz + 1;
+        }
+    }
+    top[b] = t;
+}
+__global__ __launch_bounds__(256) void k_open_dilate(const int32_t* __restrict__ top, int32_t* __restrict__ cone) {
+    __shared__ int32_t s_top[kCoarsePerAxis * kCoarsePerAxis];
+    __shared__ int32_t s_h[16];
+    for (uint32_t i = threadIdx.x; i < (uint32_t)(kCoarsePerAxis * kCoarsePerAxis); i += 256u) s_top[i] = top[i];
+    if (threadIdx.x < 16u) s_h[threadIdx.x] = kOpenNoGround;
+    __syncthreads();
+    const uint32_t slot = threadIdx.x >> 4, part = threadIdx.x & 15u;
+    const uint32_t b = blockIdx.x * 16u + slot;
+    const int bx = (int)(b & 63u), by = (int)(b >> 6);
+    int32_t h = kOpenNoGround;
+    for (uint32_t k = 0; k < 256u; k++) {
+        const uint32_t o = part * 256u + k;
+        int ax = abs((int)(o & 63u) - bx), ay = abs((int)(o >> 6) - by);
+        ax = ax < kCoarsePerAxis - ax ? ax : kCoarsePerAxis - ax; ay = ay < kCoarsePerAxis - ay ? ay : kCoarsePerAxis - ay;
+        const int ex = ax > 1 ? ax - 1 : 0, ey = ay > 1 ? ay - 1 : 0;
+        const int n = 16 * (ex * ex + ey * ey);
+        int r = (int)__builtin_sqrtf((float)n);
+        if (r * r > n) r--;
+        if ((r + 1) * (r + 1) <= n) r++;
+        const int32_t v = s_top[o] - kOpenSlope * r;
+        h = v > h ? v : h;
+    }
+    atomicMax(&s_h[slot], h);
+    __syncthreads();
+    if (threadIdx.x < 16u) cone[blockIdx.x * 16u + threadIdx.x] = s_h[threadIdx.x];
+}
+__global__ __launch_bounds__(256) void k_open_encode(const uint32_t* __restrict__ coarse, const int32_t* __restrict__ cone,
+                                                     uint32_t* __restrict__ open_map) {
+    const uint32_t w = blockIdx.x * 256u + threadIdx.x;
+    const uint32_t in = coarse[w];
+    const int z0 = 4 * (int)(w >> 9);
+    const bool low_face_zy = (w >> 9) == 0u || ((w >> 3) & 63u) == 0u;
+    uint32_t out = 0;
+    for (uint32_t k = 0; k < 8u; k++) {
+        const uint32_t n = (in >> (4u * k)) & 15u;
+        const uint32_t b = ((w << 3) | k) & 4095u;
+        const bool low_face = low_face_zy || (b & 63u) == 0u;
+        uint32_t e = n;
+        if (n >= 1u && n < kOpenBit - 1u && !low_face && z0 >= cone[b] + kOpenMarginVoxels) e = n + kOpenBit;
+        else if (n >= kOpenBit) e = kNibMixed;
+        out |= e << (4u * k);
+    }
+    open_map[w] = out;
+}
+
 __global__ __launch_bounds__(256) void k_read_box(const uint8_t* __restrict__ mine_sw, const uint32_t* __restrict__ mat_sw, int logr,
                                                   int x0, int y0, int z0, int ex, int ey, uint64_t n, uint32_t* __restrict__ mat_out,
                                                   uint8_t* __restrict__ mine_out) {
@@ -148,6 +215,15 @@
     return launch_build_maps(mine_sw, coarse, brick, logr, map_boxes_slab(logr, axis, offset), st);
 }
 
+hipError_t launch_build_open_map(const uint8_t* mine_sw, const uint32_t* coarse, uint32_t* open_map, int32_t* scratch, hipStream_t st) {
+    constexpr uint32_t kFootprints = (uint32_t)(kCoarsePerAxis * kCoarsePerAxis);
+    int32_t *top = scratch, *cone = scratch + kFootprints;
+    hipLaunchKernelGGL(k_open_heights, dim3(kFootprints / 256u), dim3(256), 0, st, mine_sw, coarse, top);
+    hipLaunchKernelGGL(k_open_dilate, dim3(kFootprints / 16u), dim3(256), 0, st, top, cone);
+    hipLaunchKernelGGL(k_open_encode, dim3((uint32_t)kCoarseWords / 256u), dim3(256), 0, st, coarse, cone, open_map);
+    return hipGetLastError();
+}
+
 hipError_t launch_check_maps(const uint8_t* mine_sw, const uint32_t* coarse, const uint32_t* brick, int logr,
                              unsigned long long* mismatches, hipStream_t st) {
     const uint32_t nbw = (logr > 8 && brick) ? (1u << (3 * (logr - 2))) / 8u : 0u;
diff --git a/raytrace_amd/render.py b/raytrace_amd/render.py
--- a/raytrace_amd/render.py
+++ b/raytrace_amd/render.py
@@ -517,6 +517,12 @@
         out = np.empty((self.cfg.height, self.cfg.width), dtype=np.uint32)
         self._check(self._lib.rt_read_history(self._h, _p(out), out.nbytes))
         return out
+
+    def read_open_map(self):
+        words = np.empty(32768, dtype=np.uint32)
+        self._check(self._lib.rt_read_open_map(self._h, _p(words), words.nbytes))
+        nib = (words[:, None] >> (4 * np.arange(8, dtype=np.uint32))[None, :]) & 15
+        return nib.astype(np.uint8).reshape(64, 64, 64)
 
     def edit_boxes_pending(self):
         boxes, over = C.c_uint32(0), C.c_uint32(0)
```

Result: no change. 54710 (-0.1%).
